# FrancisTheCat/raytracing_c

Measured on AMD Instinct MI355X. Metric: Mray/s, higher is better.
Workload: dtype f32; 1 GPU; helmet.glb 1920x1080, 256 spp, 8 bounces (BASELINE.json configs[2]); partition=single GPU

## Files before the change

### include/rt_hip.h

```cpp
#ifndef RT_HIP_H
#define RT_HIP_H

#include "rt_raytracer.h"
#include "rt_materials.h"

#ifdef __cplusplus
extern "C" {
#endif

extern char const *rt_last_error(void);
extern void        rt_clear_error(void);

extern int rt_init(int device);

extern int rt_set_devices(i32 n_devices, i32 rehearse);
extern i32 rt_device_count(void);


extern void rt_set_seed(u32 seed);
extern u32  rt_get_seed(void);


typedef struct RT_Device_Scene RT_Device_Scene;

// ... 88 lines not shown
#define RT_QUERY_MAX_RAYS ((i64)1 << 30)
extern int rt_query_closest(RT_Device_Scene *dscene, i64 n, void const *d_rays, void const *d_t_max, void *d_hits, void *d_full,
                            void *stream);
extern int rt_query_occluded(RT_Device_Scene *dscene, i64 n, void const *d_rays, void const *d_t_max, void *d_flags, void *stream);

#define RT_QUERY_SLICE ((i64)1 << 20)
extern int rt_scene_hits(Scene const *scene, i64 n, Ray const *rays, Hit *hits, i32 *triangles);
extern int rt_scene_closest(Scene const *scene, i64 n, Ray const *rays, f32 const *t_max, RT_Ray_Hit *hits);
extern int rt_scene_occluded(Scene const *scene, i64 n, Ray const *rays, f32 const *t_max, u8 *flags);

extern int rt_get_query_counters(RT_Query_Counters *out);


#define RT_FEATURE_CHANNELS 10
typedef struct { f32 *coverage, *albedo, *normal, *position; } RT_Features;

extern int rt_render_accumulate_features(RT_Device_Scene *dscene, RT_Render_Params const *params, void *d_sums, void *stream);
extern int rt_resolve_features(RT_Render_Params const *params, void const *d_sums,
                               void *d_coverage, void *d_albedo, void *d_normal, void *d_position, void *stream);
extern int rt_render_features(Scene const *scene, i32 width, i32 height, isize samples, isize max_bounces,
                              RT_Features const *out, u64 *sums);

#define RT_MOTION_CHANNELS 3
extern int rt_render_accumulate_features_motion(RT_Device_Scene *dscene, RT_Render_Params const *params, void *d_sums,
                                                void *d_motion_sums, void *stream);
extern int rt_resolve_motion(RT_Render_Params const *params, void const *d_motion_sums, void *d_motion, void *stream);
extern int rt_render_features_motion(Scene const *scene, i32 width, i32 height, isize samples, isize max_bounces,
                                     RT_Features const *out, u64 *sums, f32 *motion, u64 *motion_sums);


typedef struct {
  i32 iterations;
  f32 sigma_color, sigma_normal, sigma_position;
  i32 demodulate;
} RT_Guided_Params;

extern i64 rt_guided_work_bytes(i32 width, i32 height);
extern int rt_guided_denoise(i32 width, i32 height, RT_Guided_Params const *params, void const *d_color, void const *d_coverage,
                             void const *d_albedo, void const *d_normal, void const *d_position, void *d_out, void *d_image,
                             void *d_work, void *stream);
extern int rt_guided_denoise_host(i32 width, i32 height, RT_Guided_Params const *params, f32 const *color,
                                  RT_Features const *planes, f32 *out, u8 *image);
extern int rt_render_denoised(Scene const *scene, Image const *image, isize samples, isize max_bounces,
                              RT_Guided_Params const *params, f32 *linear_noisy, f32 *linear_denoised);


typedef struct {
  f32 alpha;
  i32 max_history;
  f32 normal_tolerance, plane_tolerance;
  i32 demodulate;
} RT_Temporal_Params;

typedef struct { f32 *color, *length, *coverage, *normal, *position; } RT_History_Planes;

extern i64 rt_temporal_history_bytes(i32 width, i32 height);
extern int rt_temporal_accumulate(i32 width, i32 height, RT_Temporal_Params const *params, Camera const *camera,
                                  Camera const *previous_camera, void const *d_color, void const *d_coverage, void const *d_albedo,
                                  void const *d_normal, void const *d_position, void const *d_history_in, void *d_history_out,
                                  void *d_out, void *d_length, void *d_image, void *stream);
extern int rt_temporal_accumulate_host(i32 width, i32 height, RT_Temporal_Params const *params, Camera const *camera,
                                       Camera const *previous_camera, f32 const *color, RT_Features const *planes,
                                       RT_History_Planes const *history_in, RT_History_Planes const *history_out, f32 *out,
                                       f32 *length, u8 *image);

typedef struct RT_History RT_History;
extern RT_History *rt_history_create(i32 width, i32 height);
extern int         rt_history_reset(RT_History *history);
extern void        rt_history_destroy(RT_History *history);
extern int         rt_history_set_motion(RT_History *history, int on);

extern int rt_render_temporal(Scene const *scene, Image const *image, isize samples, isize max_bounces, RT_History *history,
                              RT_Temporal_Params const *temporal_params, RT_Guided_Params const *guided_params, f32 *linear_noisy,
                              f32 *linear_out, f32 *length);


typedef struct { f32 sigma_normal, sigma_position; } RT_Variance_Params;

extern i64 rt_temporal_moments_bytes(i32 width, i32 height);
extern int rt_temporal_accumulate_moments(i32 width, i32 height, RT_Temporal_Params const *params, Camera const *camera,
                                          Camera const *previous_camera, void const *d_color, void const *d_coverage,
                                          void const *d_albedo, void const *d_normal, void const *d_position, void const *d_history_in,
                                          void *d_history_out, void *d_out, void *d_length, void *d_image, RT_Variance_Params const *vp,
                                          void const *d_moments_in, void *d_moments_out, void *d_variance, void *stream);
extern int rt_temporal_accumulate_moments_host(i32 width, i32 height, RT_Temporal_Params const *params, Camera const *camera,
                                               Camera const *previous_camera, f32 const *color, RT_Features const *planes,
                                               RT_History_Planes const *history_in, RT_History_Planes const *history_out, f32 *out,
                                               f32 *length, u8 *image, RT_Variance_Params const *vp, f32 const *moments_in,
                                               f32 *moments_out, f32 *variance);

extern int rt_temporal_accumulate_motion(i32 width, i32 height, RT_Temporal_Params const *params, Camera const *camera,
                                         Camera const *previous_camera, void const *d_color, void const *d_coverage,
                                         void const *d_albedo, void const *d_normal, void const *d_position, void const *d_history_in,
                                         void *d_history_out, void *d_out, void *d_length, void *d_image, RT_Variance_Params const *vp,
                                         void const *d_moments_in, void *d_moments_out, void *d_variance, void *stream,
                                         void const *d_motion);
extern int rt_temporal_accumulate_motion_host(i32 width, i32 height, RT_Temporal_Params const *params, Camera const *camera,
                                              Camera const *previous_camera, f32 const *color, RT_Features const *planes,
                                              RT_History_Planes const *history_in, RT_History_Planes const *history_out, f32 *out,
                                              f32 *length, u8 *image, RT_Variance_Params const *vp, f32 const *moments_in,
                                              f32 *moments_out, f32 *variance, f32 const *motion);

extern i64 rt_guided_variance_work_bytes(i32 width, i32 height);
extern int rt_guided_denoise_variance(i32 width, i32 height, RT_Guided_Params const *params, void const *d_color, void const *d_coverage,
                                      void const *d_albedo, void const *d_normal, void const *d_position, void *d_out, void *d_image,
                                      void *d_work, void *stream, void const *d_variance, void *d_variance_out);
extern int rt_guided_denoise_variance_host(i32 width, i32 height, RT_Guided_Params const *params, f32 const *color,
                                           RT_Features const *planes, f32 *out, u8 *image, f32 const *variance, f32 *variance_out);

extern int rt_render_svgf(Scene const *scene, Image const *image, isize samples, isize max_bounces, RT_History *history,
                          RT_Temporal_Params const *temporal_params, RT_Variance_Params const *variance_params,
                          RT_Guided_Params const *guided_params, f32 *linear_noisy, f32 *linear_out, f32 *length, f32 *variance);


typedef struct {
  f32 sigma_normal, sigma_position;
  i32 demodulate;
  i32 guide_samples;
} RT_Upsample_Params;

extern i64 rt_guided_upsample_work_bytes(i32 width, i32 height);
extern int rt_guided_upsample(i32 width, i32 height, RT_Upsample_Params const *params, void const *d_color_low,
                              void const *d_coverage_low, void const *d_albedo_low, void const *d_normal_low,
                              void const *d_position_low, void const *d_coverage, void const *d_albedo, void const *d_normal,
                              void const *d_position, void *d_out, void *d_image, void *d_work, void *stream);
extern int rt_guided_upsample_host(i32 width, i32 height, RT_Upsample_Params const *params, f32 const *color_low,
                                   RT_Features const *low, RT_Features const *full, f32 *out, u8 *image);
extern int rt_render_upsampled(Scene const *scene, Image const *image, isize samples, isize max_bounces,
                               RT_Upsample_Params const *upsample_params, RT_Guided_Params const *guided_params, f32 *linear_low,
                               f32 *linear_upsampled, f32 *linear_out);


extern int rt_render_accumulate_chunks(RT_Device_Scene *dscene, RT_Render_Params const *params, i32 n_list, i32 const *chunks,
                                       void *d_accum, void *stream);
extern int rt_adaptive_merge(i32 width, i32 height, i32 n, i32 n_list, i32 const *chunks, void *d_accum, void *d_fresh, void *d_err,
                             void *stream);
extern int rt_resolve_adaptive(i32 width, i32 height, void const *d_chunk_samples, void const *d_accum, void *d_image, void *d_linear,
                               void *d_sample_map, void *stream);

typedef struct {
  i32 min_samples;
  i32 max_samples;
  f32 threshold;
  i32 reserved;
} RT_Adaptive_Params;

extern int rt_render_adaptive(Scene const *scene, Image const *image, RT_Adaptive_Params const *ap, isize max_bounces, f32 *linear,
                              u64 *accum, i32 *chunk_samples);

extern int rt_get_counters(RT_Counters *out);
extern int rt_get_skipped_root_visits(u64 *out);
extern int rt_get_leafless_paths(u64 *out);
extern int rt_get_triangleless_paths(u64 *out);
extern int rt_get_fused_root_visits(u64 *out);
extern int rt_get_shade_taps_form(void);
extern int rt_materials_share_taps(f32 const *mats, i32 n_materials);

typedef struct {
  f32 stamp_ms, upload_ms, enqueue_ms, gpu_prep_ms, gpu_path_ms, gpu_resolve_ms, gpu_copy_ms, total_ms;
  f32 verify_ms;
  f32 gather_ms;
  i32 n_devices;
  i32 slowest_device;
} RT_Frame_Timing;
extern int rt_get_frame_timing(RT_Frame_Timing *out);

extern f32 rt_last_kernel_ms(void);

extern void rt_kernel_timing_reset(void);
extern f32  rt_kernel_timing_mean_ms(i32 *n_launches);

extern int rt_math_contract(void);


#ifdef __cplusplus
}
#endif

#endif
```

### raytracing_c_amd/csrc/rt_dev.hip.h

```cpp
#ifndef RT_DEV_HIP_H
#define RT_DEV_HIP_H

#include <hip/hip_runtime.h>
#include <stdint.h>

#include "rt_device.h"
#include "../../include/rt_math.h"

#define RT_BLOCK_WAVES 4
#define RT_BLOCK_THREADS (RT_BLOCK_WAVES * 64)

struct Ray3 {
  rt_v3 o, d;
  float inv_x, inv_y, inv_z;
  bool  fast;
};

__device__ __forceinline__ rt_v3 slab_bias3(const Ray3 &r) {
#ifdef RT_MATH_NO_FMA
  return rt_v3_make(0.0f, 0.0f, 0.0f);
#else
  float px, py, pz;
  asm volatile("v_mul_f32 %0, %1, %2" : "=v"(px) : "v"(r.o.x), "v"(r.inv_x));
  asm volatile("v_mul_f32 %0, %1, %2" : "=v"(py) : "v"(r.o.y), "v"(r.inv_y));
// ... 983 lines not shown
    emis = rt_v3_mul_add(s_emis, tint, emis);
    if (terminate) {
      done = true;
      radiance = emis;
    } else {
      dir = out_dir;
      tint = rt_v3_mul(tint, s_tint);
      float below = (rt_v3_dot(n_geo, out_dir) < 0.0f) ? 1.0f : 0.0f;
      float bias = (0.5f - below) * 2.0f * RT_EPS;
      org = rt_v3_madd(n_geo, bias, point);
    }
  }
  if (!done) {
    bounce += 1;
    if (bounce >= P.max_bounces) {
      done = true;
      radiance = emis;
    }
  }
  return done;
}

#define PH_NEED 0
#define PH_POP  1
#define PH_NODE 2
#define PH_LEAF 3
#define PH_HIT  4
#define PH_MISS 5

#define RT_PARK_FIELDS 18
#define RT_PARK_CAP 128
static_assert(RT_PARK_FIELDS * RT_PARK_CAP == RT_PARK_RECORD_DWORDS, "park slice size (rt_device.h) out of step");
#define RT_PARK_DENSE 48
#define RT_JOIN_CHOICES 4
#define RT_PYR_NUM 3
#define RT_PYR_DEN 4
#define RT_PYR_MIN 8
#define RT_STEAL_TRIES  16
#define RT_LEAF_CULL_MAX 4

__device__ __forceinline__ float *lds_at(float4 *smem, int byte_off) {
  asm volatile("" : "+s"(byte_off));
  return reinterpret_cast<float *>(reinterpret_cast<char *>(smem) + byte_off);
}
__device__ __forceinline__ int lane_now() {
  unsigned ones = ~0u;
  asm volatile("" : "+s"(ones));
  return (int)__builtin_amdgcn_mbcnt_hi(ones, __builtin_amdgcn_mbcnt_lo(ones, 0u));
}
__device__ __forceinline__ int lane_rank(unsigned long long mask) {
  return (int)__builtin_amdgcn_mbcnt_hi((uint32_t)(mask >> 32), __builtin_amdgcn_mbcnt_lo((uint32_t)mask, 0u));
}

template <int THREADS>
__device__ __forceinline__ void lds_load_nodes(float4 *smem, const float *nodes, int n_lds) {
  const float4 *g = reinterpret_cast<const float4 *>(nodes);
  for (int i = threadIdx.x; i < n_lds * RT_NODE_F4; i += THREADS) {
    int nd = i / RT_NODE_F4, q = i - nd * RT_NODE_F4;
    smem[nd * RT_LDS_NODE_F4 + q] = g[i];
  }
}

#define RT_LDS_PERM_LEVEL_F4 (RT_LDS_PERM_LEVEL_BYTES / 16)
#define RT_LDS_ACC_TILE_F4   (RT_LDS_ACC_TILE_BYTES / 16)
struct WaveLds {
  uint32_t *perm;
  unsigned long long *acc;
  int acc_off, pyr_off;
};
__device__ __forceinline__ int perm_stack_f4(int depth) { return (depth > 0 ? depth : 1) * RT_LDS_PERM_LEVEL_F4; }
__device__ __forceinline__ uint32_t *wave_perm(float4 *smem, int n_lds, int slice_f4, int wave) {
  return reinterpret_cast<uint32_t *>(smem + n_lds * RT_LDS_NODE_F4 + wave * slice_f4);
}
__device__ __forceinline__ WaveLds wave_lds(float4 *smem, int n_lds, int depth, int wave) {
  const int perm_f4 = perm_stack_f4(depth), slice_f4 = perm_f4 + RT_LDS_ACC_TILE_F4;
  const int base_f4 = n_lds * RT_LDS_NODE_F4 + __builtin_amdgcn_readfirstlane(wave) * slice_f4;
  WaveLds L;
  L.perm = wave_perm(smem, n_lds, slice_f4, wave);
  L.acc = reinterpret_cast<unsigned long long *>(reinterpret_cast<float4 *>(L.perm) + perm_f4);
  L.acc_off = (base_f4 + perm_f4) * 16;
  L.pyr_off = (base_f4 + perm_f4 - RT_LDS_PERM_LEVEL_F4) * 16;
  return L;
}
__device__ __forceinline__ void acc_tile_clear(unsigned long long *acc, const int lane) {
  acc[lane] = 0ull;
  acc[lane + 64] = 0ull;
  acc[lane + 128] = 0ull;
}
__device__ __forceinline__ void tile_add_sample(float4 *smem, const int acc_off, const int pixel, const rt_v3 radiance) {
  unsigned long long *ap = reinterpret_cast<unsigned long long *>(lds_at(smem, acc_off) + pixel * 6);
  atomicAdd(ap + 0, accum_quantize_dev(radiance.x));
  atomicAdd(ap + 1, accum_quantize_dev(radiance.y));
  atomicAdd(ap + 2, accum_quantize_dev(radiance.z));
}
#ifndef RT_SKY_ADD_GROUP
#define RT_SKY_ADD_GROUP 4
#endif
static_assert(RT_SKY_ADD_GROUP == 4 || RT_SKY_ADD_GROUP == 16 || RT_SKY_ADD_GROUP == 64, "RT_SKY_ADD_GROUP: 4, 16 or 64");
template <int CTRL>
__device__ __forceinline__ unsigned long long dpp_u64(const unsigned long long v) {
  typedef uint32_t u32x2 __attribute__((ext_vector_type(2)));
  u32x2 p = __builtin_bit_cast(u32x2, v);
  p.x = (uint32_t)__builtin_amdgcn_mov_dpp((int)p.x, CTRL, 0xF, 0xF, true);
  p.y = (uint32_t)__builtin_amdgcn_mov_dpp((int)p.y, CTRL, 0xF, 0xF, true);
  return __builtin_bit_cast(unsigned long long, p);
}
template <int CTRL>
__device__ __forceinline__ void dpp_add3_u64(unsigned long long &r, unsigned long long &g, unsigned long long &b) {
  const unsigned long long pr = dpp_u64<CTRL>(r), pg = dpp_u64<CTRL>(g), pb = dpp_u64<CTRL>(b);
  r += pr; g += pg; b += pb;
}
__device__ __forceinline__ unsigned long long rows_sum_u64(unsigned long long v) {
  typedef uint32_t u32x2 __attribute__((ext_vector_type(2)));
  u32x2 p = __builtin_bit_cast(u32x2, v);
  const auto l16 = __builtin_amdgcn_permlane16_swap(p.x, p.x, false, false), h16 = __builtin_amdgcn_permlane16_swap(p.y, p.y, false, false);
  u32x2 a = {l16[0], h16[0]}, b = {l16[1], h16[1]};
  v = __builtin_bit_cast(unsigned long long, a) + __builtin_bit_cast(unsigned long long, b);
  p = __builtin_bit_cast(u32x2, v);
  const auto l32 = __builtin_amdgcn_permlane32_swap(p.x, p.x, false, false), h32 = __builtin_amdgcn_permlane32_swap(p.y, p.y, false, false);
  a = u32x2{l32[0], h32[0]}; b = u32x2{l32[1], h32[1]};
  return __builtin_bit_cast(unsigned long long, a) + __builtin_bit_cast(unsigned long long, b);
}
template <int G>
__device__ __forceinline__ void group_sum3_u64(unsigned long long &r, unsigned long long &g, unsigned long long &b) {
  static_assert(G == 4 || G == 16 || G == 64, "group_sum3_u64: groups of 4, 16 or 64 lanes");
  dpp_add3_u64<0xB1>(r, g, b);
  dpp_add3_u64<0x4E>(r, g, b);
  if (G >= 16) {
    dpp_add3_u64<0x141>(r, g, b);
    dpp_add3_u64<0x140>(r, g, b);
  }
  if (G >= 64) { r = rows_sum_u64(r); g = rows_sum_u64(g); b = rows_sum_u64(b); }
}
__device__ __forceinline__ void lds_add_u64_noret(const uint32_t at, const unsigned long long r, const unsigned long long g,
                                                  const unsigned long long b) {
  asm volatile("ds_add_u64 %0, %1\n\tds_add_u64 %0, %2 offset:8\n\tds_add_u64 %0, %3 offset:16" : : "v"(at), "v"(r), "v"(g), "v"(b) : "memory");
}
__device__ __forceinline__ void tile_add_samples_grouped(float4 *smem, const int acc_off, const int pixel, const bool grouped, const bool has,
                                                         unsigned long long r, unsigned long long g, unsigned long long b) {
  bool adds = true;
  if (grouped) {
    group_sum3_u64<RT_SKY_ADD_GROUP>(r, g, b);
    adds = (lane_now() & (RT_SKY_ADD_GROUP - 1)) == 0;
  }
  if (adds && has) {
    const uint32_t at = (uint32_t)(uintptr_t)(__attribute__((address_space(3))) float *)lds_at(smem, acc_off) + (uint32_t)pixel * 24u;
    lds_add_u64_noret(at, r, g, b);
  }
}
#define RT_PYR_PLANE      0
#define RT_PYR_ORIGIN     16
#define RT_PYR_ROOT_POP   19
#define RT_PYR_ROOT_FUSED 20
#define RT_PYR_LEAF_CACHE 24
#define RT_PYR_NODE_CACHE 32
#define RT_PYR_CACHE_WORDS 40

__device__ __forceinline__ bool child_box_empty(float mnx, float mny, float mnz, float mxx, float mxy, float mxz) {
  return mnx == 0.0f && mny == 0.0f && mnz == 0.0f && mxx == 0.0f && mxy == 0.0f && mxz == 0.0f;
}
__device__ __forceinline__ bool child_box_empty(const float *nb) { return child_box_empty(nb[0], nb[8], nb[16], nb[24], nb[32], nb[40]); }

__device__ __forceinline__ uint32_t pyramid_cull_mask(const float4 *lds_nodes, const float *pyr, int node) {
  const int lane = lane_now();
  const float *nb = reinterpret_cast<const float *>(lds_nodes + lds_node_f4(node)) + (lane & 7);
  const float *pl = pyr + RT_PYR_PLANE + ((lane >> 3) & 3) * 4;
  const float ox = pyr[RT_PYR_ORIGIN], oy = pyr[RT_PYR_ORIGIN + 1], oz = pyr[RT_PYR_ORIGIN + 2];
  const float mnx = nb[0], mny = nb[8], mnz = nb[16], mxx = nb[24], mxy = nb[32], mxz = nb[40];
  const float nx = pl[0], ny = pl[1], nz = pl[2];
  const bool empty = child_box_empty(mnx, mny, mnz, mxx, mxy, mxz);
  const float lox = nx * (mnx - ox), hix = nx * (mxx - ox), loy = ny * (mny - oy), hiy = ny * (mxy - oy);
  const float loz = nz * (mnz - oz), hiz = nz * (mxz - oz);
  const float nearest = fminf(lox, hix) + fminf(loy, hiy) + fminf(loz, hiz);
  const float extent = fmaxf(fabsf(lox), fabsf(hix)) + fmaxf(fabsf(loy), fabsf(hiy)) + fmaxf(fabsf(loz), fabsf(hiz));
  const float coarse = fabsf(nx) * (fabsf(ox) + fmaxf(fabsf(mnx), fabsf(mxx))) + fabsf(ny) * (fabsf(oy) + fmaxf(fabsf(mny), fabsf(mxy))) +
                       fabsf(nz) * (fabsf(oz) + fmaxf(fabsf(mnz), fabsf(mxz)));
  const bool outside = empty || nearest > 1e-3f * extent + 1e-6f * coarse;
  const uint32_t m = (uint32_t)__ballot(outside);
  return (m | (m >> 8) | (m >> 16) | (m >> 24)) & 0xFFu;
}

__device__ __forceinline__ float slab_entry_ordered(const Ray3 &r, const rt_v3 &bs, const char *nbase, int k, int nx, int ny, int nz, float t_max) {
  const char *b = nbase + k * 4;
  const float sx = rt_slab_t_fast(*reinterpret_cast<const float *>(b + nx), r.o.x, r.inv_x, bs.x);
  const float bx = rt_slab_t_fast(*reinterpret_cast<const float *>(b + (96 - nx)), r.o.x, r.inv_x, bs.x);
  const float sy = rt_slab_t_fast(*reinterpret_cast<const float *>(b + 32 + ny), r.o.y, r.inv_y, bs.y);
  const float by = rt_slab_t_fast(*reinterpret_cast<const float *>(b + 32 + (96 - ny)), r.o.y, r.inv_y, bs.y);
  const float sz = rt_slab_t_fast(*reinterpret_cast<const float *>(b + 64 + nz), r.o.z, r.inv_z, bs.z);
  const float bz = rt_slab_t_fast(*reinterpret_cast<const float *>(b + 64 + (96 - nz)), r.o.z, r.inv_z, bs.z);
  const float t_minv = fmax_hw(RT_EPS, fmax_hw(sx, fmax_hw(sy, sz)));
  const float t_maxv = fmin_hw(t_max, fmin_hw(bx, fmin_hw(by, bz)));
  return (t_minv < t_maxv) ? t_minv : RT_INF;
}

#define LGM_FEW(name) do { if (AT_ROOT) LGM("rfew_" name); else LGM("nfew_" name); } while (0)
template <bool AT_ROOT = false>
__device__ __forceinline__ uint32_t node_enter_few(const Ray3 &r, const float4 *lds_nodes, int node, uint32_t surv,
                                                   float hit_t) {
  const char *nbase = reinterpret_cast<const char *>(lds_nodes + lds_node_f4(node));
  const int nx = (as_i(r.inv_x) >> 31) & 96, ny = (as_i(r.inv_y) >> 31) & 96, nz = (as_i(r.inv_z) >> 31) & 96;
  const rt_v3 bs = slab_bias3(r);
  const int n = (int)__popc(surv);
  const int k0 = (int)__builtin_ctz(surv);
  const int e0 = as_i(slab_entry_ordered(r, bs, nbase, k0, nx, ny, nz, hit_t));
  const uint32_t f0 = 1u - (((uint32_t)e0 + 0x00800000u) >> 31);
  LGM_FEW("ret1");
  if (n == 1) return (uint32_t)k0 | (f0 << 24);
  surv &= surv - 1u;
  const int k1 = (int)__builtin_ctz(surv);
  const int e1 = as_i(slab_entry_ordered(r, bs, nbase, k1, nx, ny, nz, hit_t));
  const uint32_t f1 = 1u - (((uint32_t)e1 + 0x00800000u) >> 31);
  LGM_FEW("two");
  if (n == 2) {
    const bool swap = e1 < e0;
    const uint32_t first = swap ? (uint32_t)k1 : (uint32_t)k0, second = swap ? (uint32_t)k0 : (uint32_t)k1;
    return first | (second << 3) | ((f0 + f1) << 24);
  }
  LGM_FEW("ret2");
  surv &= surv - 1u;
  const int k2 = (int)__builtin_ctz(surv);
  const int e2 = as_i(slab_entry_ordered(r, bs, nbase, k2, nx, ny, nz, hit_t));
  const uint32_t f2 = 1u - (((uint32_t)e2 + 0x00800000u) >> 31);
  int e3 = 0x7F800000, k3 = 0;
  uint32_t f3 = 0;
  LGM_FEW("four_begin");
  if (n == 4) {
    surv &= surv - 1u;
    k3 = (int)__builtin_ctz(surv);
      e3 = as_i(slab_entry_ordered(r, bs, nbase, k3, nx, ny, nz, hit_t));
    f3 = 1u - (((uint32_t)e3 + 0x00800000u) >> 31);
  }
  LGM_FEW("four_end");
  const int e[4] = {e0, e1, e2, e3};
  const int kk[4] = {k0, k1, k2, k3};
  int rank[4] = {0, 1, 2, 3};
#pragma unroll
  for (int j = 0; j < 4; j++) {
#pragma unroll
    for (int k = j + 1; k < 4; k++) {
      int kb = (int)((uint32_t)(e[k] - e[j]) >> 31);
      rank[j] += kb;
      rank[k] -= kb;
    }
  }
  uint32_t w = 0;
#pragma unroll
  for (int j = 0; j < 4; j++) w |= (uint32_t)kk[j] << (3 * rank[j]);
  return w | ((f0 + f1 + f2 + f3) << 24);
}
#undef LGM_FEW

template <bool PADDING = false>
__device__ __forceinline__ uint32_t pyramid_cull_tris(const float *leaves, const float *pyr, int g, uint32_t *padding = nullptr) {
  const int lane = lane_now();
  const float *tb = leaves + (size_t)g * 72 + (lane & 7);
  const float *pl = pyr + RT_PYR_PLANE + ((lane >> 3) & 3) * 4;
  const float ox = pyr[RT_PYR_ORIGIN], oy = pyr[RT_PYR_ORIGIN + 1], oz = pyr[RT_PYR_ORIGIN + 2];
  const float nx = pl[0], ny = pl[1], nz = pl[2];
  const float ax = tb[0], e1x = tb[8], e2x = tb[16], ay = tb[24], e1y = tb[32], e2y = tb[40], az = tb[48], e1z = tb[56], e2z = tb[64];
  const float band = 2.5f * RT_EPS * (fabsf(nx * e1x + ny * e1y + nz * e1z) + fabsf(nx * e2x + ny * e2y + nz * e2z));
  bool outside = true;
#pragma unroll
  for (int v = 0; v < 3; v++) {
    const float vx = v == 0 ? ax : (v == 1 ? ax + e1x : ax + e2x);
    const float vy = v == 0 ? ay : (v == 1 ? ay + e1y : ay + e2y);
    const float vz = v == 0 ? az : (v == 1 ? az + e1z : az + e2z);
    const float px = nx * (vx - ox), py = ny * (vy - oy), pz = nz * (vz - oz);
    const float val = px + py + pz;
    const float extent = fabsf(px) + fabsf(py) + fabsf(pz);
    const float coarse = fabsf(nx) * (fabsf(ox) + fabsf(vx)) + fabsf(ny) * (fabsf(oy) + fabsf(vy)) + fabsf(nz) * (fabsf(oz) + fabsf(vz));
    outside = outside && (val - band > 1e-3f * extent + 1e-6f * coarse);
  }
  const uint32_t m = (uint32_t)__ballot(outside);
  if (PADDING) {
    const bool zero = ax == 0.0f && e1x == 0.0f && e2x == 0.0f && ay == 0.0f && e1y == 0.0f && e2y == 0.0f && az == 0.0f && e1z == 0.0f && e2z == 0.0f;
    *padding = (uint32_t)__ballot(zero) & 0xFFu;
  }
  return (m | (m >> 8) | (m >> 16) | (m >> 24)) & 0xFFu;
}

template <bool SHORT_DIV>
__device__ __forceinline__ void tri_test_uniform(const Ray3 &r, rt_v3 a, rt_v3 edge1, rt_v3 edge2, int k, float &best, float &bu, float &bv, int &bi) {
  rt_v3 rxe2 = rt_v3_cross(r.d, edge2);
  float det = rt_v3_dot(edge1, rxe2);
  float inv_det = SHORT_DIV ? rcp_leaf(det) : 1.0f / det;
  rt_v3 s = rt_v3_sub(r.o, a);
  rt_v3 sxe1 = rt_v3_cross(s, edge1);
  float u = inv_det * rt_v3_dot(s, rxe2);
  float v = inv_det * rt_v3_dot(r.d, sxe1);
  float t = inv_det * rt_v3_dot(edge2, sxe1);
  bool miss = (u < -RT_EPS) || (u > 1.0f + RT_EPS) || (v < -RT_EPS) || (u + v > 1.0f + RT_EPS) || (t < RT_EPS);
  if (SHORT_DIV) {
    if (!miss && t < best) { best = t; bi = k; bu = u; bv = v; }
  } else {
    float dist = miss ? RT_INF : t;
    dist = (dist > 0.0f) ? dist : RT_INF;
    if (dist < best) { best = dist; bi = k; bu = u; bv = v; }
  }
}
template <bool SHORT_DIV>
__device__ __forceinline__ bool leaf_test_uniform(const RT_KParams &P, const Ray3 &r, int g, uint32_t surv, HitRec &hit) {
  float best = RT_INF, bu = 0.0f, bv = 0.0f;
  int   bi = 0;
  cfloat *lb = as_scalar_ptr(P.leaves) + (size_t)g * 72;
  while (surv) {
    const int k0 = (int)__builtin_ctz(surv);
// ... 340 lines not shown
```

### raytracing_c_amd/csrc/rt_device.h

```cpp
#ifndef RT_DEVICE_H
#define RT_DEVICE_H

#include <stdint.h>

#define RT_NODE_F4   12
#define RT_LEAF_F4   18
#define RT_TRI_F4     7
#define RT_MAT_F4     9
#define RT_MAT_FLOATS 36
#define RT_MAX_DEPTH  8

#define RT_LDS_BYTES            (160 * 1024)
#define RT_LDS_NODE_BYTES       208
#define RT_LDS_TABLE_BYTES      64
#define RT_LDS_PERM_LEVEL_BYTES 256
#define RT_LDS_ACC_TILE_BYTES   1536

#define RT_MAT_DISNEY 0
#define RT_MAT_DEBUG  1

#define RT_TILE      8
#define RT_TILE_PIX  64

#define RT_PARK_RECORD_DWORDS (18 * 128)
enum {
  RT_CNT_PATHS = 0, RT_CNT_RAYS, RT_CNT_NODES, RT_CNT_LEAVES, RT_CNT_SHADES, RT_CNT_BG, RT_CNT_TEXTURED,
  RT_CNT_SKIPPED_ROOT,
  RT_CNT_LEDGER,
  RT_CNT_LEAFLESS = 136,
  RT_CNT_FUSED_ROOT,
  RT_CNT_TRIANGLELESS,
  RT_N_COUNTERS
};
#define RT_CNT_LEDGER_SLOTS (RT_CNT_LEAFLESS - RT_CNT_LEDGER)



typedef struct {
  uint32_t offset;
  int32_t  width, height, stride;
} RT_DTexture;
#define RT_TEX_TILE_INDEX(x, y, tpr) ((((y) >> 2) * (tpr) + ((x) >> 2)) * 16 + (((y) & 3) << 2) + ((x) & 3))

typedef struct RT_KView {
  float    cam[3][4];
  float    focal_length;
  uint32_t seed;
  uint32_t pad[2];
} RT_KView;

typedef struct {
  const float    *nodes;
  const float    *leaves;
  const float    *tris;
  const float    *mats;
  const RT_DTexture *textures;
  const uint32_t *texels;
  int32_t depth;
  int32_t last_row_offset;
  int32_t bg_texture;
  int32_t n_nodes;
  float cam[3][4];
  float focal_length;
  float inv_width, inv_height, aspect;
  int32_t width, height, samples, max_bounces;
  int32_t sample_first, sample_end;
  uint32_t seed;
  int32_t chunks_x, n_chunks;
  int32_t rank, world, n_local_chunks;
  int32_t shared_taps;
  int32_t unused_pad[2];
  int32_t sched_thresh;
  int32_t n_lds_nodes;
  unsigned long long *accum;
  unsigned long long *counters;
  uint32_t *work_head;
  const int32_t *local_chunks;
  const uint32_t *order;
  uint32_t *tile_cost;
  unsigned long long *wave_times;
  uint32_t *tile_next;
  uint32_t *open_groups;
  int32_t n_tiles;
  int32_t chunk_shift;
  int32_t n_chunks_tile;
  int32_t n_sample_blocks;
  int32_t drain_thresh;
  int32_t grab_max;
  uint32_t *park;
  int32_t short_div;
  int32_t pyr_nodes;
  uint32_t *wf_hit0;
  uint32_t *wf_hit;
  uint32_t *wf_ray[2];
  uint32_t *wf_cnt_hit0, *wf_cnt_hit, *wf_cnt_ray[2];
  uint32_t *wf_ctl;
  int32_t wf_soft_chunks;
  int32_t wf_bounce;
  int32_t wf_n_waves;
  const RT_KView *views;
  int32_t n_views;
  int32_t tiles_per_view;
  int32_t pixels_per_view;
} RT_KParams;

typedef struct {
  const float *rays;
  const float *t_max;
  float       *hits;
  uint8_t     *flags;
  uint32_t    *head;
  unsigned long long *counters;
  int32_t      n;
  int32_t      grab;
  int32_t      exit_lanes;
} RT_QParams;
enum { RT_QCNT_RAYS = 0, RT_QCNT_HITS, RT_QCNT_NODES, RT_QCNT_LEAVES, RT_QUERY_COUNTERS };
#define RT_HIT_DWORDS     22

typedef struct {
  unsigned long long *sums;
  uint32_t    *head;
  int32_t      n_units;
  int32_t      grab;
  int32_t      tiles_x;
  int32_t      shift;
  int32_t      n_sample_blocks;
  int32_t      units_per_tile;
} RT_FParams;

typedef struct {
  float r[3][3];
  float t[3];
  float focal_length;
} RT_TCamera;
typedef struct {
  RT_TCamera cur, prev;
  int32_t width, height;
  float   half_w, half_h;
  float   aspect;
  float   tn2, tp2;
  float   alpha;
  float   max_history;
  int32_t demodulate;
  int32_t tiles_x;
} RT_TParams;

typedef struct {
  const float *color, *coverage, *albedo, *normal, *position;
} RT_Frame;

#define WF_CHUNK        256
#define WF_HIT0_FIELDS  9
#define WF_HIT_FIELDS   5
#define WF_RAY_FIELDS   15
#define WF_CTL_STRIDE   16
enum {
  WF_HIT0_ALLOC = 0, WF_HIT0_HEAD, WF_HIT_ALLOC, WF_HIT_HEAD, WF_RAY0_ALLOC, WF_RAY0_HEAD, WF_RAY1_ALLOC, WF_RAY1_HEAD,
  WF_STOPPED,
  WF_DONE_WAVES,
  WF_N_CTL
};

#endif
```

### raytracing_c_amd/csrc/rt_kernels.hip

```cpp

#include "rt_dev.hip.h"


#ifdef RT_LEDGER
#define RT_LEDGER_WAVES 8192
__device__ uint32_t g_ledger[RT_LEDGER_WAVES * RT_LEDGER_ROW];
__global__ void rt_ledger_reduce_kernel(unsigned long long *counters) {
  const int slot = threadIdx.x;
  if (slot >= LG_N || slot >= RT_LEDGER_ROW) return;
  unsigned long long sum = 0ull;
  for (int w = 0; w < RT_LEDGER_WAVES; w++) sum += g_ledger[w * RT_LEDGER_ROW + slot];
  counters[RT_CNT_LEDGER + slot] = sum;
}
#endif

template <int WAVES, bool LDSN, int MIN_WAVES_PER_SIMD, bool SHORT_DIV, bool VIEWS, bool SHARED_TAPS>
__global__ __launch_bounds__(WAVES * 64, MIN_WAVES_PER_SIMD) void rt_path_kernel_stream(RT_KParams P) {
  extern __shared__ float4 smem[];
  const int lane = threadIdx.x & 63;
  const int wave = threadIdx.x >> 6;
  const int n_lds = LDSN ? P.n_lds_nodes : 0;
  const float4 *lds_nodes = smem;
  const WaveLds L = wave_lds(smem, n_lds, P.depth, wave);
  unsigned long long *acc = L.acc;
  const int acc_off = L.acc_off, pyr_off = L.pyr_off;

#ifdef RT_LEDGER
  uint32_t *lg = g_ledger + (size_t)__builtin_amdgcn_readfirstlane((int)blockIdx.x * WAVES + wave) * RT_LEDGER_ROW;
  const unsigned long long lg_wave_t0 = __builtin_amdgcn_s_memtime();
#if RT_LEDGER >= 2
  unsigned long long lg_drain_t0 = 0ull;
#endif
#endif
  pow24_lds_init((int)threadIdx.x);
  if (LDSN) {
    LGT0();
    lds_load_nodes<WAVES * 64>(smem, P.nodes, n_lds);
    __syncthreads();
    LGT1(LG_CYC_COPY);
  } else {
    __syncthreads();
  }

  acc_tile_clear(acc, lane);

  if (LDSN) {
    uint32_t *pw = reinterpret_cast<uint32_t *>(lds_at(smem, pyr_off));
    bool populated = false;
    if (lane_now() < 8 && cold_args()->n_lds_nodes > 0 && cold_args()->depth > 0) {
      populated = !child_box_empty(lds_at(smem, 0) + lane_now());
    }
    const uint32_t pm = (uint32_t)__ballot(populated) & 0xFFu;
#ifdef RT_ROOT_AT_NODE_BLOCKS
    if (lane_now() == 0) { pw[RT_PYR_ROOT_POP] = 0u; pw[RT_PYR_ROOT_FUSED] = 0u; }
#else
    if (lane_now() == 0) { pw[RT_PYR_ROOT_POP] = __popc(pm) <= 4 ? pm : 0u; pw[RT_PYR_ROOT_FUSED] = 0u; }
#endif
  }

  uint32_t w_paths = 0, w_rays = 0, w_nodes = 0, w_leaves = 0, w_shades = 0, w_bgs = 0, w_tex = 0;
  const unsigned long long t_wave_start = cold_args()->wave_times ? __builtin_amdgcn_s_memrealtime() : 0ull;
  uint32_t n_tiles_done = 0;
  unsigned long long t_last_grab = 0ull;

  const int shift = P.chunk_shift;
  const int unit_paths = 2 << shift;
  const uint32_t n_chunks_tile = (uint32_t)P.n_chunks_tile;
  const int leaf_level = P.depth - 1;
  const int thresh = P.sched_thresh;
  const int drain_thresh = P.drain_thresh;
  const int pyr_nodes = LDSN ? P.pyr_nodes : 0;
  const int wave_id = (int)blockIdx.x * WAVES + wave;

  bool queue_open = true;
  int  steal_tries = 0;

  for (;;) {
    LGT0();
    LGM("tile_begin");
    int tile_idx = queue_open ? take_queue_tile(lane, queue_open) : -1;
    if (tile_idx < 0) {
      if (steal_tries >= RT_STEAL_TRIES) break;
      steal_tries += 1;
      LG(LG_JOIN_X, 1);
      tile_idx = join_open_tile(lane, wave_id, steal_tries, n_chunks_tile LG_ARG);
      if (tile_idx < 0) break;
    }

    int tile_x0, tile_y0;
    RT_KViewP vrec = nullptr;
    if (!tile_origin<VIEWS>(lane, tile_idx, n_chunks_tile, tile_x0, tile_y0, vrec)) continue;
    bool tile_root_miss = false;
    if (leaf_level >= 0) {
      typename CamSrc<VIEWS>::type S;
      if constexpr (VIEWS) S = vrec; else S = cold_args();
      tile_root_miss = tile_pyramid(S, P.nodes, smem, pyr_off, lane, tile_x0, tile_y0);
    }
    int n_list = 0;
    int ll_levels = leaf_level, ll_nodes = pyr_nodes, ll_leaf0 = P.last_row_offset;
    asm volatile("" : "+s"(ll_levels), "+s"(ll_nodes), "+s"(ll_leaf0));
    if (ll_levels >= 1 && ll_nodes > 0 && !tile_root_miss) n_list = leafless_walk(smem, lds_nodes, pyr_off, ll_levels, ll_nodes, ll_leaf0, cold_args()->leaves);
    const uint32_t rays_before = w_rays;
    LG(LG_TILE_X, 1);
    LGM("tile_end");
    LGT1(LG_CYC_TILE);

    int   pix = 0, bounce = 0;
    uint32_t rng = 0;
    Ray3  ray;
    ray_setup(ray, rt_v3_make(0, 0, 0), rt_v3_make(0, 0, 1));
    rt_v3 tint = rt_v3_make(1, 1, 1), emis = rt_v3_make(0, 0, 0);
    TravState T = RT_TRAV_IDLE;

    bool tile_open = true;
    TileUnits U;
    tile_units_init(U, queue_open);
    int  n_parked = 0;
    uint32_t *park = cold_args()->park;

    if ((tile_root_miss || n_list > 0) && cold_args()->max_bounces > 0) {
      RT_KArgs A = cold_args();
      typename CamSrc<VIEWS>::type S;
      if constexpr (VIEWS) S = vrec; else S = A;
      const int width = A->width, height = A->height, sample_first = A->sample_first, sample_end = A->sample_end;
      const uint32_t n_sb = (uint32_t)A->n_sample_blocks, gmax = (uint32_t)A->grab_max;
      PrimaryParams PP;
      primary_params(PP, S, A);
      ShadeParamsLds SP;
      shade_params(SP, A, false);
      uint32_t *tile_next = A->tile_next, *open_groups = A->open_groups;
      uint32_t n_sky = 0;
      const uint32_t *list = leafless_list(smem, pyr_off, ll_levels);
      const uint32_t list_entry = (n_list > 1 && lane_now() < n_list) ? list[RT_LL_ENTRY + (lane_now() & 31)] : 0u;
      for (;;) {
        if (U.c_next >= U.c_end) {
          if (U.u_cur + 1u < U.u_end) {
            U.u_cur += 1u;
          } else {
            uint32_t u0 = 0;
            if (lane == 0) u0 = atomicAdd(&tile_next[tile_idx], U.grab);
            u0 = (uint32_t)__builtin_amdgcn_readfirstlane((int)u0);
            if (u0 >= n_chunks_tile) { tile_open = false; break; }
            U.u_cur = u0;
            U.u_end = u0 + U.grab < n_chunks_tile ? u0 + U.grab : n_chunks_tile;
            if (U.u_end == n_chunks_tile && lane == 0) atomicSub(&open_groups[tile_idx >> 6], 1u);
            if (t_wave_start) t_last_grab = __builtin_amdgcn_s_memrealtime();
            LG(LG_GRAB_X, 1);
            const uint32_t left = n_chunks_tile - U.u_end;
            U.grab = left >= 8u * gmax ? gmax : (left >= 8u && gmax >= 2u ? 2u : 1u);
            U.took_any = true;
          }
          unit_decode(U, tile_x0, tile_y0, shift, unit_paths, n_sb, sample_first, width, height);
          continue;
        }
#ifndef RT_SKY_PATHS
#define RT_SKY_PATHS 1
#endif
        LGM("sky_begin");
        LGT0();
        const int avail = U.c_end - U.c_next;
        const int take = avail < 64 * RT_SKY_PATHS ? avail : 64 * RT_SKY_PATHS;
        const int l = lane_now();
        bool valid[RT_SKY_PATHS];
        int  pxs[RT_SKY_PATHS];
        rt_v3 dirs[RT_SKY_PATHS];
        Ray3 rs[RT_SKY_PATHS];
        bool slow = false;
#pragma unroll
        for (int q = 0; q < RT_SKY_PATHS; q++) {
          const int kq = l + 64 * q;
          const int k = U.c_next + kq;
          pxs[q] = k >> shift;
          const int sm = U.c_s0 + (k & ((1 << shift) - 1));
          const int x = U.c_x0 + pxs[q];
          valid[q] = kq < take && x < width && sm < sample_end;
          rt_v3 o = rt_v3_make(0, 0, 0);
          dirs[q] = rt_v3_make(0, 0, 1);
          if (valid[q]) primary_ray(PP, x, U.c_y, sm, o, dirs[q]);
          ray_setup<SHORT_DIV>(rs[q], o, dirs[q]);
          slow = slow || (valid[q] && !rs[q].fast);
        }
        if (__ballot(slow) != 0ull) break;
        uint32_t nv = 0;
        uint32_t e = (uint32_t)__builtin_amdgcn_readlane((int)list_entry, 1);
        if ((int)e < 0) {
#pragma unroll
          for (int q = 0; q < RT_SKY_PATHS; q++) {
            const Ray3 &r = rs[q];
            const int nx = (as_i(r.inv_x) >> 31) & 96, ny = (as_i(r.inv_y) >> 31) & 96, nz = (as_i(r.inv_z) >> 31) & 96;
            const rt_v3 bs = slab_bias3(r);
            uint32_t entered = valid[q] ? 1u : 0u;
            int i = 1;
            if (q > 0) e = (uint32_t)__builtin_amdgcn_readlane((int)list_entry, 1);
            do {
              const char *cb = reinterpret_cast<const char *>(lds_nodes) + (e & 0xFFFFFu);
              const float t = slab_entry_ordered(r, bs, cb, 0, nx, ny, nz, RT_INF);
              const uint32_t in = ((entered >> ((e >> 20) & 31u)) & 1u) & (t < RT_INF ? 1u : 0u);
              entered |= in << i;
              const uint32_t n_in = (uint32_t)__popcll(__ballot(in != 0u));
              if (e & RT_LL_GROUP) w_leaves += n_in;
              else w_nodes += n_in;
              i += 1;
              e = (uint32_t)__builtin_amdgcn_readlane((int)list_entry, i);
            } while ((int)e < 0);
          }
        }
#pragma unroll
        for (int q = 0; q < RT_SKY_PATHS; q++) {
          unsigned long long qr = 0ull, qg = 0ull, qb = 0ull;
          if (valid[q]) {
            const rt_v3 bg = background_lookup(SP, dirs[q]);
            const rt_v3 radiance = rt_v3_mul_add(bg, rt_v3_make(1, 1, 1), rt_v3_make(0, 0, 0));
            qr = accum_quantize_dev(radiance.x); qg = accum_quantize_dev(radiance.y); qb = accum_quantize_dev(radiance.z);
          }
          tile_add_samples_grouped(smem, acc_off, U.c_pix0 + pxs[q], U.c_end >= 2 * RT_SKY_ADD_GROUP, valid[q], qr, qg, qb);
          nv += (uint32_t)__popcll(__ballot(valid[q]));
        }
        w_paths += nv; w_rays += nv; w_nodes += nv; w_bgs += nv;
        n_sky += nv;
        LG(LG_SKY_X, 1); LG(LG_SKY_L, nv);
        U.c_next += take;
        LGT1(LG_CYC_SKY);
        LGM("sky_end");
      }
      if (n_sky != 0u && lane == 0) atomicAdd(cold_args()->counters + (tile_root_miss ? RT_CNT_SKIPPED_ROOT : RT_CNT_LEAFLESS), (unsigned long long)n_sky);
      if (n_sky != 0u && (__ballot((list_entry & RT_LL_GROUP) != 0u) & ~1ull) != 0ull && lane == 0)
        atomicAdd(cold_args()->counters + RT_CNT_TRIANGLELESS, (unsigned long long)n_sky);
    }

    for (;;) {
      {
        LGT0();
        LGM("s_begin");
        LG(LG_S_ITER, 1);
        LaneCounters cn;
        cn.rays = cn.nodes = cn.leaves = cn.shades = cn.bgs = cn.textured = cn.paths = 0;
        bool  done = false, start = false, fresh = false;
        rt_v3 radiance = rt_v3_make(0, 0, 0);
        rt_v3 org = ray.o, dir = ray.d;
        RT_KArgs A = cold_args();
        typename PathShadeParams<SHARED_TAPS>::type SP;
        shade_params(SP, A, true);
#ifdef RT_LEDGER
        { const int n_env = (int)__popcll(__ballot(T.phase == PH_MISS)); LG(LG_ENV_X, n_env != 0); LG(LG_ENV_L, n_env); }
#endif
        LGM("env_begin");
        if (T.phase == PH_MISS) {
          cn.bgs = 1;
          rt_v3 bg = background_lookup(SP, dir);
          radiance = rt_v3_mul_add(bg, tint, emis);
          done = true;
        }
        LGM("env_end");
        bool shade_now = true;
        if (park) {
          const unsigned long long mHit = __ballot(T.phase == PH_HIT);
          const unsigned long long mIdle = __ballot(T.phase == PH_NEED) | __ballot(T.phase == PH_MISS);
          const int h = (int)__popcll(mHit), f = (int)__popcll(mIdle);
          const int back = n_parked < f ? n_parked : f;
          uint32_t *pk = park + (size_t)__builtin_amdgcn_readfirstlane(wave_id) * (RT_PARK_FIELDS * RT_PARK_CAP);
          if (!tile_open || h + back >= RT_PARK_DENSE || n_parked + h > RT_PARK_CAP) {
            if (back > 0) {
              LG(LG_PLOAD_X, 1); LG(LG_PLOAD_L, back);
              LGM("pload_begin");
              if (done) {
                tile_add_sample(smem, acc_off, pix, radiance);
                T.phase = PH_NEED;
                done = false;
              }
              const int rank = lane_rank(mIdle);
              if (T.phase == PH_NEED && rank < back) {
                const uint32_t *q = pk + (n_parked - 1 - rank);
                uint32_t v[RT_PARK_FIELDS];
                __builtin_amdgcn_fence(__ATOMIC_ACQUIRE, "wavefront");
#pragma unroll
                for (int i = 0; i < RT_PARK_FIELDS; i++)
                  v[i] = __hip_atomic_load(q + i * RT_PARK_CAP, __ATOMIC_RELAXED, __HIP_MEMORY_SCOPE_AGENT);
                T.hit.t = as_f((int)v[0]); T.hit.tri = (int)v[1]; T.hit.u = as_f((int)v[2]); T.hit.v = as_f((int)v[3]);
                org = rt_v3_make(as_f((int)v[4]), as_f((int)v[5]), as_f((int)v[6]));
                dir = rt_v3_make(as_f((int)v[7]), as_f((int)v[8]), as_f((int)v[9]));
                tint = rt_v3_make(as_f((int)v[10]), as_f((int)v[11]), as_f((int)v[12]));
                emis = rt_v3_make(as_f((int)v[13]), as_f((int)v[14]), as_f((int)v[15]));
                rng = v[16]; pix = (int)(v[17] & 63u); bounce = (int)(v[17] >> 6);
                T.phase = PH_HIT;
              }
              n_parked -= back;
              LGM("pload_end");
            }
          } else if (h > 0) {
            LG(LG_PSTORE_X, 1); LG(LG_PSTORE_L, h);
            LGM("pstore_begin");
            shade_now = false;
            const int rank = lane_rank(mHit);
            if (T.phase == PH_HIT) {
              uint32_t *q = pk + (n_parked + rank);
              const uint32_t v[RT_PARK_FIELDS] = {(uint32_t)as_i(T.hit.t), (uint32_t)T.hit.tri, (uint32_t)as_i(T.hit.u), (uint32_t)as_i(T.hit.v),
                                                  (uint32_t)as_i(org.x), (uint32_t)as_i(org.y), (uint32_t)as_i(org.z),
                                                  (uint32_t)as_i(dir.x), (uint32_t)as_i(dir.y), (uint32_t)as_i(dir.z),
                                                  (uint32_t)as_i(tint.x), (uint32_t)as_i(tint.y), (uint32_t)as_i(tint.z),
                                                  (uint32_t)as_i(emis.x), (uint32_t)as_i(emis.y), (uint32_t)as_i(emis.z),
                                                  rng, (uint32_t)pix | ((uint32_t)bounce << 6)};
#pragma unroll
              for (int i = 0; i < RT_PARK_FIELDS; i++) q[i * RT_PARK_CAP] = v[i];
              __builtin_amdgcn_fence(__ATOMIC_RELEASE, "wavefront");
              T.phase = PH_NEED;
            }
            n_parked += h;
            LGM("pstore_end");
          }
        }
#ifdef RT_LEDGER
        { const int n_sh = (int)__popcll(__ballot(T.phase == PH_HIT && shade_now)); LG(LG_SHADE_X, n_sh != 0); LG(LG_SHADE_L, n_sh); }
#endif
        LGM("shade_begin");
        if (T.phase == PH_HIT && shade_now) {
          done = shade_hit(SP, T.hit, org, dir, tint, emis, rng, bounce, cn, radiance);
          start = !done;
        }
        LGM("shade_end");
#ifdef RT_LEDGER
        { const int n_acc = (int)__popcll(__ballot(done)); LG(LG_ACCUM_X, n_acc != 0); LG(LG_ACCUM_L, n_acc); }
#endif
        LGM("accum_begin");
        if (done) {
          tile_add_sample(smem, acc_off, pix, radiance);
          T.phase = PH_NEED;
        }
        LGM("accum_end");
        w_shades += (uint32_t)__popcll(__ballot(cn.shades != 0));
        w_tex += (uint32_t)__popcll(__ballot(cn.textured != 0));
        w_bgs += (uint32_t)__popcll(__ballot(cn.bgs != 0));

        if (tile_open) {
          NewPath np = {0, 0, 0, 0};
          const bool got = regen_paths(T.phase, np, SP.max_bounces > 0, U, tile_open, false, lane, tile_idx, n_chunks_tile, tile_x0, tile_y0,
                                       shift, unit_paths, t_wave_start, t_last_grab, w_paths LG_ARG);
          if (!tile_open) LGD0((int)__popcll(__ballot(T.phase != PH_NEED || got)) + n_parked);
          const int gx = np.x, gy = np.y, gs = np.sample, width = A->width;
#ifdef RT_LEDGER
          { const int n_pr = (int)__popcll(__ballot(got)); LG(LG_PRIM_X, n_pr != 0); LG(LG_PRIM_L, n_pr); LG(LG_REGEN_L, n_pr); }
#endif
          LGM("prim_begin");
          if (got) {
            typename CamSrc<VIEWS>::type S;
            if constexpr (VIEWS) S = vrec; else S = A;
            pix = np.pix;
            bounce = 0;
            rng = rt_path_seed(S->seed, (uint32_t)(gx + gy * width), (uint32_t)gs);
            PrimaryParams PP;
            primary_params(PP, S, A);
            primary_ray(PP, gx, gy, gs, org, dir);
            tint = rt_v3_make(1, 1, 1);
            emis = rt_v3_make(0, 0, 0);
            start = true;
            fresh = true;
          }
          LGM("prim_end");
        }
        bool skip_root = false;
#ifdef RT_LEDGER
        { const int n_st = (int)__popcll(__ballot(start)); LG(LG_START_X, n_st != 0); LG(LG_START_L, n_st); }
#endif
        LGM("start_begin");
        if (start) {
          ray_setup<SHORT_DIV>(ray, org, dir);
          trav_start(T, leaf_level, P.last_row_offset);
          T.cur = (LDSN && ray.fast && reinterpret_cast<const uint32_t *>(lds_at(smem, pyr_off))[RT_PYR_ROOT_POP] != 0u) ? 1u : 0u;
          skip_root = fresh && tile_root_miss && ray.fast;
          if (skip_root) T.phase = PH_MISS;
        }
        LGM("start_end");
        w_rays += (uint32_t)__popcll(__ballot(start));
        {
          const uint32_t n_skip = (uint32_t)__popcll(__ballot(skip_root));
          w_nodes += n_skip;
          if (n_skip != 0u && lane == 0) atomicAdd(cold_args()->counters + RT_CNT_SKIPPED_ROOT, (unsigned long long)n_skip);
        }
        LGM("s_end");
        LGT1(LG_CYC_S);
      }

      const int n_trav0 = (int)__popcll(__ballot(T.phase == PH_NODE || T.phase == PH_LEAF));
      if (n_trav0 == 0) {
        if (__any(T.phase == PH_MISS)) continue;
        if (n_parked > 0 || __any(T.phase == PH_HIT)) continue;
        if (!tile_open) break;
        continue;
      }

      if (LDSN) {
        const bool at_root = T.phase == PH_NODE && T.level < 0 && T.cur != 0u;
        const int n_root = (int)__popcll(__ballot(at_root));
        if (n_root != 0) {
          LGM("root_begin");
          LG(LG_ROOTF_X, 1); LG(LG_ROOTF_L, n_root);
          uint32_t *pw = reinterpret_cast<uint32_t *>(lds_at(smem, pyr_off));
          const uint32_t w_pop = pw[RT_PYR_ROOT_POP], w_cull = pw[RT_PYR_NODE_CACHE];
          uint32_t rsurv = (uint32_t)__builtin_amdgcn_readfirstlane((int)w_pop);
          w_nodes += (uint32_t)n_root;
          if (lane_now() == 0) {
            const uint32_t at = (uint32_t)(uintptr_t)(__attribute__((address_space(3))) uint32_t *)(pw + RT_PYR_ROOT_FUSED);
            asm volatile("ds_add_u32 %0, %1" : : "v"(at), "v"((uint32_t)n_root) : "memory");
          }
          if (__ballot(at_root && bounce != 0) == 0ull) {
            const uint32_t ce = (uint32_t)__builtin_amdgcn_readfirstlane((int)w_cull);
            if ((ce >> 8) == 1u) rsurv &= ~ce;
          }
          if (at_root) {
            T.level = 0;
            T.cur = rsurv ? node_enter_few<true>(ray, lds_nodes, 0, rsurv, RT_INF) : 0u;
            if (T.cur >> 24) {
              T.child = 1 + (int)(T.cur & 7u);
              T.cur = ((T.cur >> 3) & 0x1FFFFFu) | (((T.cur >> 24) - 1u) << 24);
              T.phase = (leaf_level == 0) ? PH_LEAF : PH_NODE;
            } else {
              T.level = -1;
              T.phase = PH_MISS;
            }
          }
          LGM("root_end");
        }
      }

      const TravWave W = {smem, lds_nodes, L.perm, n_lds, pyr_nodes, pyr_off, leaf_level, lane};
      traversal_blocks<LDSN, SHORT_DIV, true>(P, W, ray, bounce == 0, T, tile_open ? thresh : drain_thresh, n_trav0, w_nodes, w_leaves LG_ARG);
    }

    LGD1();
    LGM("flush_begin");
    if (U.took_any) {
      LGT0();
      LG(LG_FLUSH_X, 1);
      RT_KArgs A = cold_args();
      unsigned long long *frame = A->accum;
      if constexpr (VIEWS) frame += (size_t)(vrec - (RT_KViewP)A->views) * (size_t)A->pixels_per_view * 3;
      flush_tile(acc, lane, tile_x0, tile_y0, frame, tile_idx, w_rays - rays_before);
      if (LDSN && lane == 0) {
        uint32_t *pw = reinterpret_cast<uint32_t *>(lds_at(smem, pyr_off));
        const uint32_t n_fused = pw[RT_PYR_ROOT_FUSED];
        pw[RT_PYR_ROOT_FUSED] = 0u;
        if (n_fused != 0u) atomicAdd(A->counters + RT_CNT_FUSED_ROOT, (unsigned long long)n_fused);
      }
      steal_tries = 0;
      n_tiles_done += 1;
      LGT1(LG_CYC_FLUSH);
    }
  }
  RT_KArgs A = cold_args();
  unsigned long long *wave_times = A->wave_times, *counters = A->counters;
  if (wave_times && lane == 0 && wave_id < 65536) {
    wave_times[wave_id * 3 + 0] = t_wave_start;
    wave_times[wave_id * 3 + 1] = __builtin_amdgcn_s_memrealtime();
    wave_times[wave_id * 3 + 2] = ((t_last_grab - t_wave_start) << 16) | (n_tiles_done & 0xFFFFu);
  }

  if (lane == 0) {
    atomicAdd(counters + RT_CNT_PATHS, (unsigned long long)w_paths);
    atomicAdd(counters + RT_CNT_RAYS, (unsigned long long)w_rays);
    atomicAdd(counters + RT_CNT_NODES, (unsigned long long)w_nodes);
    atomicAdd(counters + RT_CNT_LEAVES, (unsigned long long)w_leaves);
    atomicAdd(counters + RT_CNT_SHADES, (unsigned long long)w_shades);
    atomicAdd(counters + RT_CNT_BG, (unsigned long long)w_bgs);
    atomicAdd(counters + RT_CNT_TEXTURED, (unsigned long long)w_tex);
#ifdef RT_LEDGER
    LG(LG_CYC_WAVE, (uint32_t)((__builtin_amdgcn_s_memtime() - lg_wave_t0) >> 4));
#endif
  }
}

__global__ void rt_resolve_kernel(int width, int height, int samples, int chunks_x, const int32_t *local_chunks,
                                  int n_local_chunks, const unsigned long long *accum,
                                  uint8_t *tiles, uint8_t *image, float *linear) {
  int idx = blockIdx.x * blockDim.x + threadIdx.x;
  if (idx >= n_local_chunks * 1024) return;
  int lchunk = idx >> 10, p = idx & 1023;
  int chunk = local_chunks[lchunk];
  int x = (chunk % chunks_x) * 32 + (p & 31);
  int y = (chunk / chunks_x) * 32 + (p >> 5);
  uint8_t rgb[3] = {0, 0, 0};
  if (x < width && y < height) {
    size_t pix = (size_t)y * width + x;
#pragma unroll
    for (int c = 0; c < 3; c++) {
      float lin = rt_accum_resolve(accum[pix * 3 + c], (uint32_t)samples);
      if (linear) linear[pix * 3 + c] = lin;
      rgb[c] = rt_encode_u8(lin);
      if (image) image[pix * 3 + c] = rgb[c];
    }
  }
// ... 440 lines not shown
```

### raytracing_c_amd/csrc/rt_launch.cpp

```cpp

#include "rt_host.h"

static std::atomic<int> g_taps_form{-1};

int check_params(RT_Render_Params const *p) {
  if (!p) return rt_fail("render params are NULL");
  if (p->width <= 0 || p->height <= 0) return rt_fail("image size %dx%d is invalid", p->width, p->height);
  if ((int64_t)p->width * p->height > (int64_t)1 << 28) return rt_fail("image %dx%d is too large", p->width, p->height);
  if (p->samples <= 0) return rt_fail("samples must be positive (got %d)", p->samples);
  if (p->max_bounces < 0) return rt_fail("max_bounces must be >= 0 (got %d)", p->max_bounces);
  if (p->world <= 0 || p->rank < 0 || p->rank >= p->world) return rt_fail("rank %d / world %d is invalid", p->rank, p->world);
  if (p->sample_first < 0 || p->sample_count < 0 || p->sample_first + p->sample_count > p->samples)
    return rt_fail("sample range [%d, +%d) outside [0, %d)", p->sample_first, p->sample_count, p->samples);
  return 0;
}

int check_image_size(const char *who, i32 width, i32 height) {
  if (width <= 0 || height <= 0) return rt_fail("%s: image size %dx%d is invalid", who, width, height);
  if ((int64_t)width * height > RT_MAX_PIXELS) return rt_fail("%s: image %dx%d is too large (more than 2^28 pixels)", who, width, height);
  return 0;
}

int check_views(i32 n_views, RT_View const *views, i32 width, i32 height, const char *who) {
  if (n_views <= 0) return rt_fail("%s: n_views must be positive (got %d)", who, n_views);
// ... 91 lines not shown
  if (batch) {
    K->n_views = nv;
    K->tiles_per_view = K->n_local_chunks * 16;
    K->pixels_per_view = p->width * p->height;
  }
  return 0;
}

static void launch_geometry(const Device &D, const RT_Device_Scene *d, RT_KParams &K, int *wg_waves, int *smem) {
  const int64_t paths = (int64_t)K.n_tiles * 64 * (int64_t)(K.sample_end - K.sample_first);
  int64_t per_slot = paths / ((int64_t)D.num_cus * 16 * 64);
  if (K.depth == 0) per_slot /= 4;
  *wg_waves = per_slot < 12 ? 8 : (per_slot < 40 ? 12 : 16);
  int v = knob_int("RT_WG_WAVES", 0);
  if (v == 8 || v == 12 || v == 16) *wg_waves = v;
  LdsSplit S = lds_split(d, K.depth, *wg_waves, RT_LDS_ACC_TILE_BYTES, 1, true);
  S.cap(knob_int("RT_LDS_NODES", -1));
  K.n_lds_nodes = S.n_lds_nodes;
  *smem = S.smem;
}

static int schedule_feedback(LaunchState &L, RT_KParams &K, const uint32_t **cost_prev) {
  K.order = nullptr;
  K.tile_cost = nullptr;
  *cost_prev = nullptr;
  if (knob_is("RT_ORDER", "identity") || K.n_tiles <= 0) return 0;
  const int n_tiles = K.n_tiles;
  uint64_t key = 1469598103934665603ull;
  auto mix = [&key](const void *ptr, size_t n) {
    const unsigned char *b = (const unsigned char *)ptr;
    for (size_t i = 0; i < n; i++) { key ^= b[i]; key *= 1099511628211ull; }
  };
  int32_t ids[6] = {K.width, K.height, K.rank, K.world, K.max_bounces, n_tiles};
  mix(ids, sizeof ids);
  if (L.sched_tiles != n_tiles) {
    L.cost[0].reset(); L.cost[1].reset(); L.order.reset();
    L.sched_tiles = 0;
    L.sched_valid = false;
    HIP_TRY(L.cost[0].grow((size_t)n_tiles));
    HIP_TRY(L.cost[1].grow((size_t)n_tiles));
    HIP_TRY(L.order.grow((size_t)n_tiles));
    L.sched_tiles = n_tiles;
  }
  if (L.sched_valid && L.sched_key == key) {
    *cost_prev = L.cost[L.sched_cur ^ 1];
    K.order = L.order;
  }
  K.tile_cost = L.cost[L.sched_cur];
  L.sched_cur ^= 1;
  L.sched_key = key;
  L.sched_valid = true;
  return 0;
}

static int upload_view_table(LaunchState &L, RT_KParams &K, ViewBatch const *batch, hipStream_t stream) {
  const int nv = batch->n;
  HIP_TRY(L.views.grow((size_t)nv));
  HIP_TRY(L.views_host.grow((size_t)nv));
  if (!L.views_copied) HIP_TRY(L.views_copied.ensure(hipEventDisableTiming));
  else HIP_TRY(hipEventSynchronize(L.views_copied));
  for (int v = 0; v < nv; v++) {
    RT_KView &r = L.views_host[v];
    memset(&r, 0, sizeof r);
    camera_rows(r.cam, &batch->views[v].camera);
    r.focal_length = batch->views[v].camera.focal_length;
    r.seed = batch->views[v].seed;
  }
  HIP_TRY(hipMemcpyAsync(L.views, L.views_host, (size_t)nv * sizeof(RT_KView), hipMemcpyHostToDevice, stream));
  HIP_TRY(hipEventRecord(L.views_copied, stream));
  K.views = L.views;
  return 0;
}

int stage_chunk_list(ChunkListStage &S, ChunkList const &list, hipStream_t stream, const int32_t **d_list) {
  if (!S.copied) HIP_TRY(S.copied.ensure(hipEventDisableTiming));
  else HIP_TRY(hipEventSynchronize(S.copied));
  if (S.dev && S.dev.cap < (size_t)list.n) HIP_TRY(hipStreamSynchronize(stream));
  HIP_TRY(S.dev.grow((size_t)list.n));
  HIP_TRY(S.host.grow((size_t)list.n));
  if (list.n > 0) {
    memcpy(S.host.get(), list.chunks, (size_t)list.n * sizeof(int32_t));
    HIP_TRY(hipMemcpyAsync(S.dev, S.host, (size_t)list.n * sizeof(int32_t), hipMemcpyHostToDevice, stream));
    HIP_TRY(hipEventRecord(S.copied, stream));
  }
  *d_list = S.dev;
  return 0;
}

int render_accumulate_locked(Device &D, RT_Device_Scene *d, Camera const *cam, RT_Render_Params const *p, void *d_accum,
                             hipStream_t stream, hipEvent_t ev_prep, int launch_state, ViewBatch const *batch, ChunkList const *list) {
  if (ensure_device(D) != 0) return -1;
  if (check_params(p) != 0) return -1;
  if (!d || !d_accum) return rt_fail("rt_render_accumulate: NULL scene or accumulation buffer");
  if (d->dev != &D) return rt_fail("rt_render_accumulate: the scene was uploaded to another device");
  if (batch && check_views(batch->n, batch->views, p->width, p->height, "view batch") != 0) return -1;
  if (list && (batch || launch_state != RT_ADAPTIVE_STATE || p->rank != 0 || p->world != 1 ||
               check_chunk_list("chunk list", p->width, p->height, list->n, list->chunks) != 0))
    return rt_fail("rt_render_accumulate: a chunk list needs rank 0 of 1, no view batch, its own launch state and a valid list");
  const int nv = batch ? batch->n : 1;
  RT_KParams K;
  if (fill_kparams(D, &K, d, cam, p, d_accum, batch, list) != 0) return -1;
  if (launch_state < 0 || launch_state > RT_ADAPTIVE_STATE) return rt_fail("rt_render_accumulate: launch state %d out of range", launch_state);
  if (!list && launch_state == RT_ADAPTIVE_STATE) return rt_fail("rt_render_accumulate: launch state %d serves chunk lists only", launch_state);
  LaunchState &L = d->ls[launch_state];
  HIP_TRY(L.counters.grow(RT_N_COUNTERS));
  HIP_TRY(L.work_head.grow(16));
  K.counters = L.counters;
  K.work_head = L.work_head;
  D.last_counters = L.counters;
  bool wavefront = false;
#ifdef RT_DIAG_VARIANTS
  wavefront = g_pipeline.load() == 1 || knob_is("RT_PIPELINE", "wf");
#endif
  if (batch && wavefront) return rt_fail("view batch: a batch of views needs the tile-stream path kernel (the wavefront pipeline is set)");

  int wg_waves, smem;
  launch_geometry(D, d, K, &wg_waves, &smem);
  int waves_per_cu = knob_int("RT_WAVES_PER_CU", 0);
  if (waves_per_cu <= 0) waves_per_cu = wg_waves;
  K.sched_thresh = knob_int("RT_SCHED_THRESH", 48);
  if (K.sched_thresh < 1 || K.sched_thresh > 64) K.sched_thresh = 48;
  K.drain_thresh = knob_int("RT_DRAIN_THRESH", K.sched_thresh);
  if (K.drain_thresh < 1 || K.drain_thresh > 64) K.drain_thresh = K.sched_thresh;

  const uint32_t *cost_prev = nullptr;
  K.order = nullptr;
  K.tile_cost = nullptr;
  if (!list && schedule_feedback(L, K, &cost_prev) != 0) return -1;

  const int n_samples = K.sample_end - K.sample_first;
  const int cs = p->slab > 0 ? p->slab : 64;
  int cshift = 0;
  while ((1 << cshift) < cs && (1 << cshift) < n_samples) cshift++;
  K.chunk_shift = cshift;
  K.n_sample_blocks = (n_samples + (1 << cshift) - 1) >> cshift;
  K.n_chunks_tile = 32 * K.n_sample_blocks;
  const int tiles_room = list ? K.n_chunks * 16 : K.n_tiles;
  if (L.tile_next_n < tiles_room) {
    L.tile_next_n = 0;
    HIP_TRY(L.tile_next.grow((size_t)tiles_room + (size_t)((tiles_room + 63) / 64)));
    L.tile_next_n = tiles_room;
  }
  K.tile_next = L.tile_next;
  K.open_groups = L.tile_next + L.tile_next_n;
  const int64_t n_units = (int64_t)K.n_tiles * K.n_chunks_tile;
  int n_waves = D.num_cus * waves_per_cu;
  if ((int64_t)n_waves > n_units) n_waves = (int)n_units;
  K.grab_max = (cshift >= 6 || (int64_t)K.n_tiles < (int64_t)2 * n_waves) ? 1 : 2;
  {
    int v = knob_int("RT_GRAB", 0);
    if (v == 1 || v == 2 || v == 4) K.grab_max = v;
  }
  K.pyr_nodes = knob_int("RT_PYRAMID", 1) ? K.n_lds_nodes : 0;
  float cam_max = 0.0f;
  for (int v = 0; v < nv; v++)
    for (int i = 0; i < 3; i++)
      for (int j = 0; j < 3; j++) {
        float m = fabsf(batch ? batch->views[v].camera.view_matrix.rows[i][j] : K.cam[i][j]);
        if (!(m <= cam_max)) cam_max = m;
      }
  K.short_div = (d->max_edge <= 0x1p38f && cam_max <= 0x1p16f) ? 1 : 0;
  if (knob_int("RT_SHORT_DIV", 1) == 0) K.short_div = 0;
  K.shared_taps = (d->shared_taps && knob_int("RT_SHARED_TAPS", 1) != 0) ? 1 : 0;
  K.park = nullptr;
  if (!wavefront && knob_int("RT_PARK", 1) != 0 && K.max_bounces < (1 << 26)) {
    const int grid_waves = (n_waves + wg_waves - 1) / wg_waves * wg_waves;
    const size_t slice_dwords = RT_PARK_RECORD_DWORDS;
    HIP_TRY(L.park.grow((size_t)grid_waves * slice_dwords));
    K.park = L.park;
  }

  K.views = nullptr;
  if (batch && upload_view_table(L, K, batch, stream) != 0) return -1;
  if (list && stage_chunk_list(L.list, *list, stream, &K.local_chunks) != 0) return -1;

  {
    int rc2 = rt_launch_prepare(K.n_tiles, K.tile_next, K.open_groups, L.counters, L.work_head, K.tile_cost, cost_prev,
                                cost_prev ? L.order : nullptr, stream);
    if (rc2 != 0) return rt_fail("prepare kernel launch failed: %s", hipGetErrorString((hipError_t)rc2));
  }
  if (ev_prep) HIP_TRY(hipEventRecord(ev_prep, stream));
  if (n_units == 0) return 0;

  K.wave_times = nullptr;
  if (knob_set("RT_WAVE_TIMES")) {
    HIP_TRY(D.ws.wave_times.grow((size_t)65536 * 3));
    HIP_TRY(hipMemsetAsync(D.ws.wave_times, 0, (size_t)65536 * 3 * 8, stream));
    K.wave_times = D.ws.wave_times;
    if (n_waves > 65536) n_waves = 65536;
    D.ws.wave_times_n = n_waves;
  }

  size_t slot = D.ws.n_timed % RT_MAX_TIMED;
  if (slot >= D.ws.ev0.size()) {
    D.ws.ev0.emplace_back();
    D.ws.ev1.emplace_back();
  }
  HIP_TRY(D.ws.ev0[slot].ensure());
  HIP_TRY(D.ws.ev1[slot].ensure());
  HIP_TRY(hipEventRecord(D.ws.ev0[slot], stream));
#ifdef RT_DIAG_VARIANTS
  if (wavefront) {
    if (launch_wavefront(D, d, K, stream) != 0) return -1;
  } else
#endif
  {
    int rc = rt_launch_path_kernel(&K, n_waves, smem, wg_waves, stream);
    if (rc != 0) return rt_fail("path kernel launch failed: %s", hipGetErrorString((hipError_t)rc));
    g_taps_form.store(K.shared_taps);
  }
  HIP_TRY(hipEventRecord(D.ws.ev1[slot], stream));
  D.ws.n_timed += 1;
  return 0;
}

extern "C" int rt_set_camera(RT_Device_Scene *dscene, Camera const *camera) {
  if (!dscene || !camera) return rt_fail("rt_set_camera: NULL argument");
  Device &D = *dscene->dev;
  std::lock_guard<std::mutex> lock(D.mutex);
  D.cameras[dscene] = *camera;
  return 0;
}

extern "C" int rt_render_accumulate(RT_Device_Scene *dscene, RT_Render_Params const *params, void *d_accum,
                                    void *stream) {
  if (!dscene) return rt_fail("rt_render_accumulate: NULL scene or accumulation buffer");
  Device &D = *dscene->dev;
  std::lock_guard<std::mutex> lock(D.mutex);
  DeviceGuard guard(D);
  auto it = D.cameras.find(dscene);
  if (it == D.cameras.end()) return rt_fail("rt_render_accumulate: no camera set for this scene (rt_set_camera)");
  forget_multi_counters();
  return render_accumulate_locked(D, dscene, &it->second, params, d_accum, (hipStream_t)stream);
}

extern "C" int rt_render_accumulate_chunks(RT_Device_Scene *dscene, RT_Render_Params const *params, i32 n_list, i32 const *chunks,
                                           void *d_accum, void *stream) {
  const char *who = "rt_render_accumulate_chunks";
  if (!dscene || !d_accum) return rt_fail("%s: NULL scene or accumulation buffer", who);
  if (check_params(params) != 0) return -1;
  if (params->world != 1 || params->rank != 0)
    return rt_fail("%s: a chunk list replaces the partition: rank 0 of world 1 only (got %d of %d)", who, params->rank, params->world);
  if (check_chunk_list(who, params->width, params->height, n_list, chunks) != 0) return -1;
  Device &D = *dscene->dev;
  std::lock_guard<std::mutex> lock(D.mutex);
  DeviceGuard guard(D);
  auto it = D.cameras.find(dscene);
  if (it == D.cameras.end()) return rt_fail("%s: no camera set for this scene (rt_set_camera)", who);
  forget_multi_counters();
  ChunkList list;
  list.n = n_list;
  list.chunks = chunks;
  return render_accumulate_locked(D, dscene, &it->second, params, d_accum, (hipStream_t)stream, nullptr, RT_ADAPTIVE_STATE, nullptr, &list);
}

extern "C" int rt_render_accumulate_views(RT_Device_Scene *dscene, RT_Render_Params const *params, i32 n_views,
                                          RT_View const *views, void *d_accum, void *stream) {
  if (!dscene || !d_accum) return rt_fail("rt_render_accumulate_views: NULL scene or accumulation buffer");
  if (check_params(params) != 0) return -1;
  if (check_views(n_views, views, params->width, params->height, "rt_render_accumulate_views") != 0) return -1;
  Device &D = *dscene->dev;
  std::lock_guard<std::mutex> lock(D.mutex);
  DeviceGuard guard(D);
  forget_multi_counters();
  ViewBatch batch;
  batch.n = n_views;
  batch.views = views;
  return render_accumulate_locked(D, dscene, &views[0].camera, params, d_accum, (hipStream_t)stream, nullptr, RT_VIEWS_STATE, &batch);
}

int resolve_on(Device &D, RT_Render_Params const *p, void const *d_accum, void *d_tiles, void *d_image, void *d_linear,
               hipStream_t stream) {
  if (check_params(p) != 0) return -1;
  if (!d_accum) return rt_fail("rt_resolve: NULL accumulation buffer");
  int chunks_x = (p->width + RT_CHUNK_SIZE - 1) / RT_CHUNK_SIZE;
  const int32_t *d_list = nullptr;
  int n_local = 0;
  if (device_chunk_list(D, p->width, p->height, p->rank, p->world, &d_list, &n_local) != 0) return -1;
  int rc = rt_launch_resolve(p->width, p->height, p->samples, chunks_x, d_list, n_local,
                             (const unsigned long long *)d_accum, (uint8_t *)d_tiles, (uint8_t *)d_image,
                             (float *)d_linear, stream);
  if (rc != 0) return rt_fail("resolve kernel launch failed: %s", hipGetErrorString((hipError_t)rc));
  return 0;
}

extern "C" int rt_resolve(RT_Render_Params const *p, void const *d_accum, void *d_tiles, void *d_image,
                          void *d_linear, void *stream) {
  Device &D = dev0();
  {
    std::lock_guard<std::mutex> lock(D.mutex);
    if (ensure_device(D) != 0) return -1;
  }
  return resolve_on(D, p, d_accum, d_tiles, d_image, d_linear, (hipStream_t)stream);
}

int untile_on(Device &D, i32 width, i32 height, i32 world, void const *d_all_tiles, void *d_image, hipStream_t stream) {
  if (width <= 0 || height <= 0 || world <= 0 || !d_all_tiles || !d_image) return rt_fail("rt_untile: bad arguments");
  int chunks_x = (width + RT_CHUNK_SIZE - 1) / RT_CHUNK_SIZE;
  const int32_t *d_table = nullptr;
  int n_chunks = 0;
  if (!partition_args_ok(width, height, world)) return rt_fail("rt_untile: bad arguments");
  if (device_owner_table(D, width, height, world, &d_table, &n_chunks) != 0) return -1;
  int rc = rt_launch_untile(width, height, chunks_x, n_chunks, d_table, (const uint8_t *)d_all_tiles,
                            (uint8_t *)d_image, stream);
  if (rc != 0) return rt_fail("untile kernel launch failed: %s", hipGetErrorString((hipError_t)rc));
  return 0;
}

extern "C" int rt_untile(i32 width, i32 height, i32 world, void const *d_all_tiles, void *d_image, void *stream) {
  Device &D = dev0();
  {
    std::lock_guard<std::mutex> lock(D.mutex);
    if (ensure_device(D) != 0) return -1;
  }
  return untile_on(D, width, height, world, d_all_tiles, d_image, (hipStream_t)stream);
}

int ensure_ws_buffers(Workspace &W, int width, int height, size_t tiles_bytes, size_t all_tiles_bytes, bool want_linear) {
  const size_t pixels = (size_t)width * height;
  HIP_TRY(W.accum.grow(pixels * 3));
  HIP_TRY(W.image.grow(pixels * 3));
  if (want_linear) HIP_TRY(W.linear.grow(pixels * 3));
  if (tiles_bytes) HIP_TRY(W.tiles.grow(tiles_bytes));
  if (all_tiles_bytes) HIP_TRY(W.all_tiles.grow(all_tiles_bytes));
  for (DevEvent &e : W.ev_frame) HIP_TRY(e.ensure());
  return 0;
}

int copy_image_out(Image const *image, const uint8_t *d_image, int width, int height, hipStream_t stream) {
  size_t pixels = (size_t)width * height;
  if (!image->pixels.data) return 0;
  if (image->components == 3 && image->stride == image->width) {
    HIP_TRY(hipMemcpyAsync(image->pixels.data, d_image, pixels * 3, hipMemcpyDeviceToHost, stream));
    HIP_TRY(hipStreamSynchronize(stream));
  } else {
    std::vector<uint8_t> tmp(pixels * 3);
    HIP_TRY(hipMemcpy(tmp.data(), d_image, pixels * 3, hipMemcpyDeviceToHost));
    for (isize y = 0; y < image->height; y++)
      for (isize x = 0; x < image->width; x++)
        for (int c = 0; c < 3; c++)
          image->pixels.data[image->components * (x + y * image->stride) + c] = tmp[((size_t)y * width + x) * 3 + c];
  }
  return 0;
}

static int get_counter(const char *who, int index, u64 *out) {
  if (!out) return rt_fail("%s: NULL", who);
  Device &D = dev0();
  std::lock_guard<std::mutex> lock(D.mutex);
  if (ensure_device(D) != 0) return -1;
  unsigned long long c[RT_N_COUNTERS];
  if (read_counters(D, c) != 0) return -1;
  *out = c[index];
  return 0;
}

extern "C" int rt_get_skipped_root_visits(u64 *out) { return get_counter("rt_get_skipped_root_visits", RT_CNT_SKIPPED_ROOT, out); }

extern "C" int rt_get_leafless_paths(u64 *out) { return get_counter("rt_get_leafless_paths", RT_CNT_LEAFLESS, out); }

extern "C" int rt_get_triangleless_paths(u64 *out) { return get_counter("rt_get_triangleless_paths", RT_CNT_TRIANGLELESS, out); }

extern "C" int rt_get_fused_root_visits(u64 *out) { return get_counter("rt_get_fused_root_visits", RT_CNT_FUSED_ROOT, out); }

extern "C" int rt_get_shade_taps_form(void) { return g_taps_form.load(); }

int read_counters(Device &D, unsigned long long c[RT_N_COUNTERS]) {
  HIP_TRY(hipDeviceSynchronize());
  if (!D.last_counters) { memset(c, 0, RT_N_COUNTERS * sizeof(unsigned long long)); return 0; }
  HIP_TRY(hipMemcpy(c, D.last_counters, RT_N_COUNTERS * sizeof(unsigned long long), hipMemcpyDeviceToHost));
  return 0;
}

extern "C" int rt_get_counters(RT_Counters *out) {
  if (!out) return rt_fail("rt_get_counters: NULL");
  {
    std::lock_guard<std::mutex> lk(g_multi_mutex);
    if (g_multi_counters_valid) { *out = g_multi_counters; return 0; }
  }
  Device &D = dev0();
  std::lock_guard<std::mutex> lock(D.mutex);
  if (ensure_device(D) != 0) return -1;
  unsigned long long c[RT_N_COUNTERS];
  if (read_counters(D, c) != 0) return -1;
  out->paths = c[RT_CNT_PATHS];
  out->rays = c[RT_CNT_RAYS];
  out->node_visits = c[RT_CNT_NODES];
  out->leaf_visits = c[RT_CNT_LEAVES];
  out->shades = c[RT_CNT_SHADES];
  out->backgrounds = c[RT_CNT_BG];
  out->textured = c[RT_CNT_TEXTURED];
  return 0;
}

static float timed_slot_ms(Workspace &W, size_t slot) {
  if (hipEventSynchronize(W.ev1[slot]) != hipSuccess) return -1.0f;
  return event_ms(W.ev0[slot], W.ev1[slot]);
}

extern "C" f32 rt_last_kernel_ms(void) {
  Device &D = dev0();
  std::lock_guard<std::mutex> lock(D.mutex);
  if (!D.ready || D.ws.n_timed == 0) return -1.0f;
  DeviceGuard guard(D);
  return timed_slot_ms(D.ws, (D.ws.n_timed - 1) % RT_MAX_TIMED);
}

extern "C" void rt_kernel_timing_reset(void) {
  Device &D = dev0();
  std::lock_guard<std::mutex> lock(D.mutex);
  D.ws.n_timed = 0;
}

extern "C" f32 rt_kernel_timing_mean_ms(i32 *n_launches) {
  Device &D = dev0();
  std::lock_guard<std::mutex> lock(D.mutex);
  size_t n = D.ws.n_timed < RT_MAX_TIMED ? D.ws.n_timed : RT_MAX_TIMED;
  if (n_launches) *n_launches = (i32)n;
  if (!D.ready || n == 0) return -1.0f;
  DeviceGuard guard(D);
  double sum = 0.0;
  for (size_t i = 0; i < n; i++) {
    float ms = timed_slot_ms(D.ws, i);
    if (ms < 0.0f) return -1.0f;
    sum += ms;
  }
  return (float)(sum / (double)n);
}
```

### raytracing_c_amd/csrc/rt_tile.hip.h

```cpp
#ifndef RT_TILE_HIP_H
#define RT_TILE_HIP_H

typedef const RT_KView __attribute__((address_space(4))) *RT_KViewP;
template <bool VIEWS> struct CamSrc { typedef RT_KArgs type; };
template <> struct CamSrc<true> { typedef RT_KViewP type; };

__device__ __forceinline__ int take_queue_tile(const int lane, bool &queue_open) {
  RT_KArgs A = cold_args();
  uint32_t pos = 0;
  if (lane == 0) pos = atomicAdd(A->work_head, 1u);
  pos = (uint32_t)__builtin_amdgcn_readfirstlane((int)pos);
  const uint32_t *order = A->order;
  if (pos < (uint32_t)A->n_tiles) return order ? (int)order[pos] : (int)pos;
  queue_open = false;
  return -1;
}

__device__ __forceinline__ int join_open_tile(const int lane, const int wave_id, const int steal_tries, const uint32_t n_chunks_tile,
                                              uint32_t *lg = nullptr) {
  LGT0();
  int tile_idx = -1;
  RT_KArgs A = cold_args();
  const int n_tiles = A->n_tiles;
  const uint32_t *open_groups = A->open_groups, *tile_next = A->tile_next;
  const int n_groups = (n_tiles + 63) >> 6;
  const int g_rounds = (n_groups + 63) >> 6;
  const uint32_t hsh = ((uint32_t)wave_id * 2654435761u + (uint32_t)steal_tries * 40503u) >> 8;
  const int g_start = (int)(hsh % (uint32_t)g_rounds);
  for (int i = 0; i < g_rounds && tile_idx < 0; i++) {
    int r = g_start + i;
    if (r >= g_rounds) r -= g_rounds;
    int g = r * 64 + lane;
    uint32_t n_open = 0;
    if (g < n_groups) n_open = __hip_atomic_load(&open_groups[g], __ATOMIC_RELAXED, __HIP_MEMORY_SCOPE_AGENT);
    unsigned long long gm = __ballot(n_open != 0u);
    while (gm && tile_idx < 0) {
      int nth = (int)((hsh >> 6) % (uint32_t)__popcll(gm));
      unsigned long long m = gm;
      for (int k = 0; k < nth; k++) m &= m - 1ull;
      int gl = (int)__builtin_ctzll(m);
      gm &= ~(1ull << gl);
      int cand = (r * 64 + gl) * 64 + lane;
      uint32_t taken = 0xFFFFFFFFu;
      if (cand < n_tiles) taken = __hip_atomic_load(&tile_next[cand], __ATOMIC_RELAXED, __HIP_MEMORY_SCOPE_AGENT);
      unsigned long long open = __ballot(taken < n_chunks_tile);
      if (open) {
        const int n_open_tiles = (int)__popcll(open);
        int best = 0;
        uint32_t best_taken = 0xFFFFFFFFu;
#pragma unroll
        for (int c = 0; c < RT_JOIN_CHOICES; c++) {
          int nt = (int)(((hsh >> 12) * (uint32_t)(2 * c + 1) + (uint32_t)c * 7u) % (uint32_t)n_open_tiles);
          unsigned long long mm = open;
          for (int k = 0; k < nt; k++) mm &= mm - 1ull;
          const int pk_lane = (int)__builtin_ctzll(mm);
          const uint32_t tk = (uint32_t)__builtin_amdgcn_readlane((int)taken, pk_lane);
          if (tk < best_taken) { best_taken = tk; best = pk_lane; }
        }
        tile_idx = cand - lane + best;
      }
    }
  }
  LGT1(LG_CYC_JOIN);
  return tile_idx;
}

template <bool VIEWS>
__device__ __forceinline__ bool tile_origin(const int lane, const int tile_idx, const uint32_t n_chunks_tile, int &tile_x0, int &tile_y0,
                                            RT_KViewP &vrec) {
  RT_KArgs A = cold_args();
  int vt = tile_idx;
  if constexpr (VIEWS) {
    const int tu = __builtin_amdgcn_readfirstlane(tile_idx);
    const uint32_t view = (uint32_t)tu / (uint32_t)A->tiles_per_view;
    vt = tu - (int)view * A->tiles_per_view;
    vrec = (RT_KViewP)A->views + view;
  }
  const int lchunk = vt >> 4, sub = vt & 15;
  const int chunk = A->local_chunks[lchunk];
  const int chunks_x = A->chunks_x;
  tile_x0 = (chunk % chunks_x) * 32 + (sub & 3) * 8;
  tile_y0 = (chunk / chunks_x) * 32 + (sub >> 2) * 8;
  if (tile_x0 < A->width && tile_y0 < A->height) return true;
  if (lane == 0) {
    uint32_t old = atomicMax(&A->tile_next[tile_idx], n_chunks_tile);
    if (old < n_chunks_tile) atomicSub(&A->open_groups[tile_idx >> 6], 1u);
  }
  return false;
}
__device__ __forceinline__ bool tile_origin(const int lane, const int tile_idx, const uint32_t n_chunks_tile, int &tile_x0, int &tile_y0) {
  RT_KViewP no_view = nullptr;
  return tile_origin<false>(lane, tile_idx, n_chunks_tile, tile_x0, tile_y0, no_view);
}

template <class CAM>
__device__ __forceinline__ bool tile_pyramid(const CAM S, const float *nodes, float4 *smem, const int pyr_off, const int lane,
                                             const int tile_x0, const int tile_y0) {
  RT_KArgs A = cold_args();
  const float m = 0.05f;
  const float ux0 = ((float)tile_x0 - 0.5f - m) * 2.0f * A->inv_width - 1.0f;
  const float ux1 = ((float)tile_x0 + 7.5f + m) * 2.0f * A->inv_width - 1.0f;
  const float uy0 = ((float)tile_y0 - 0.5f - m) * 2.0f * A->inv_height - 1.0f;
  const float uy1 = ((float)tile_y0 + 7.5f + m) * 2.0f * A->inv_height - 1.0f;
  const float asp = A->aspect, fl = S->focal_length;
  rt_v3 c[4];
#pragma unroll
  for (int q = 0; q < 4; q++) {
    float cx = ((q == 1 || q == 2) ? ux1 : ux0) * asp, cy = -((q >= 2) ? uy1 : uy0), cz = -fl;
    c[q] = rt_v3_make(S->cam[0][0] * cx + S->cam[0][1] * cy + S->cam[0][2] * cz,
                      S->cam[1][0] * cx + S->cam[1][1] * cy + S->cam[1][2] * cz,
                      S->cam[2][0] * cx + S->cam[2][1] * cy + S->cam[2][2] * cz);
  }
  const rt_v3 o = rt_v3_make(S->cam[0][3], S->cam[1][3], S->cam[2][3]);
  rt_v3 pn[4];
#pragma unroll
  for (int q = 0; q < 4; q++) {
    rt_v3 n = rt_v3_cross(c[q], c[(q + 1) & 3]);
    if (rt_v3_dot(n, c[(q + 2) & 3]) > 0.0f) n = rt_v3_scale(n, -1.0f);
    pn[q] = n;
  }
  float *pyr = lds_at(smem, pyr_off);
  if (lane == 0) {
#pragma unroll
    for (int q = 0; q < 4; q++) { pyr[RT_PYR_PLANE + q * 4 + 0] = pn[q].x; pyr[RT_PYR_PLANE + q * 4 + 1] = pn[q].y; pyr[RT_PYR_PLANE + q * 4 + 2] = pn[q].z; }
    pyr[RT_PYR_ORIGIN] = o.x; pyr[RT_PYR_ORIGIN + 1] = o.y; pyr[RT_PYR_ORIGIN + 2] = o.z;
  }
  if (lane < RT_PYR_CACHE_WORDS) reinterpret_cast<uint32_t *>(pyr)[RT_PYR_LEAF_CACHE + lane] = 0u;
  bool may_hit = false;
  if (lane < 8) {
    const float *nb = nodes + lane;
    rt_v3 lo = rt_v3_make(nb[0] - o.x, nb[8] - o.y, nb[16] - o.z);
    rt_v3 hi = rt_v3_make(nb[24] - o.x, nb[32] - o.y, nb[40] - o.z);
    bool outside = child_box_empty(nb);
#pragma unroll
    for (int q = 0; q < 4; q++) {
      rt_v3 n = pn[q];
      float lox = n.x * lo.x, hix = n.x * hi.x, loy = n.y * lo.y, hiy = n.y * hi.y, loz = n.z * lo.z, hiz = n.z * hi.z;
      float nearest = fminf(lox, hix) + fminf(loy, hiy) + fminf(loz, hiz);
      float extent = fmaxf(fabsf(lox), fabsf(hix)) + fmaxf(fabsf(loy), fabsf(hiy)) + fmaxf(fabsf(loz), fabsf(hiz));
      float coarse = fabsf(n.x) * (fabsf(o.x) + fmaxf(fabsf(nb[0]), fabsf(nb[24]))) + fabsf(n.y) * (fabsf(o.y) + fmaxf(fabsf(nb[8]), fabsf(nb[32]))) +
                     fabsf(n.z) * (fabsf(o.z) + fmaxf(fabsf(nb[16]), fabsf(nb[40])));
      if (nearest > 1e-3f * extent + 1e-6f * coarse) outside = true;
    }
    may_hit = !outside;
  }
  return __ballot(may_hit) == 0ull;
}

#define RT_LL_MAX   32
#define RT_LL_ENTRY 0
#define RT_LL_NODE  RT_LL_MAX
#define RT_LL_GROUP 0x40000000u
static_assert(2 * RT_LL_MAX * 4 <= RT_LDS_PERM_LEVEL_BYTES && RT_LL_MAX <= 32, "the list is one row of the perm stack, `entered` one word");
__device__ __forceinline__ uint32_t *leafless_list(float4 *smem, const int pyr_off, const int levels) {
  return reinterpret_cast<uint32_t *>(lds_at(smem, pyr_off) - levels * (RT_LDS_PERM_LEVEL_BYTES / 4));
}
__device__ __forceinline__ int leafless_walk(float4 *smem, const float4 *lds_nodes, const int pyr_off, const int levels, const int n_nodes,
                                             const int leaf0, const float *leaves) {
  const float *pyr = lds_at(smem, pyr_off);
  uint32_t *list = leafless_list(smem, pyr_off, levels);
  int n_list = 1;
  for (int head = 0; head < n_list; head++) {
    const int nd = head ? __builtin_amdgcn_readfirstlane((int)list[RT_LL_NODE + head]) : 0;
    if (nd >= leaf0) continue;
    const uint32_t surv = 0xFFu & ~pyramid_cull_mask(lds_nodes, pyr, nd);
    if (lane_now() == 0) reinterpret_cast<uint32_t *>(lds_at(smem, pyr_off))[RT_PYR_NODE_CACHE + (nd & 31)] = ((uint32_t)(nd + 1) << 8) | (0xFFu & ~surv);
    if (surv) {
      const int ns = (int)__popc(surv);
      const bool groups = 8 * nd + 1 >= leaf0;
      if ((!groups && 8 * nd + 8 >= n_nodes) || ns > 4 || n_list + ns > RT_LL_MAX) return 0;
      if (groups) {
        for (uint32_t m = surv; m; m &= m - 1u) {
          const int g = 8 * nd + 1 + (int)__builtin_ctz(m) - leaf0;
          if ((uint32_t)g >= 0x800000u) return 0;
          uint32_t padding = 0u;
          const uint32_t cull = pyramid_cull_tris<true>(leaves, pyr, g, &padding);
          if (lane_now() == 0) reinterpret_cast<uint32_t *>(lds_at(smem, pyr_off))[RT_PYR_LEAF_CACHE + (g & 7)] = ((0x800000u | (uint32_t)g) << 8) | cull;
          if ((0xFFu & ~(cull | padding)) != 0u) return 0;
        }
      }
      const int k = lane_now();
      if (k < 8 && ((surv >> k) & 1u)) {
        const int at = n_list + (int)__popc(surv & ((1u << k) - 1u));
        list[RT_LL_ENTRY + at] = (uint32_t)(nd * RT_LDS_NODE_BYTES + k * 4) | ((uint32_t)head << 20) | (groups ? RT_LL_GROUP : 0u) | 0x80000000u;
        list[RT_LL_NODE + at] = (uint32_t)(8 * nd + 1 + k);
      }
      n_list += ns;
    }
  }
  return n_list;
}

struct TileUnits {
  uint32_t u_cur, u_end, grab;
  int  c_next, c_end;
  int  c_x0, c_y, c_pix0, c_s0;
  bool took_any;
};
__device__ __forceinline__ void tile_units_init(TileUnits &U, const bool queue_open) {
  U.c_next = U.c_end = U.c_x0 = U.c_y = U.c_pix0 = U.c_s0 = 0;
  U.u_cur = U.u_end = 0;
  U.grab = queue_open ? (uint32_t)cold_args()->grab_max : 1u;
  U.took_any = false;
}

__device__ __forceinline__ bool grab_units(const int lane, const int tile_idx, const uint32_t n_chunks_tile, uint32_t *tile_next,
                                           uint32_t *open_groups, const uint32_t gmax, TileUnits &U, const unsigned long long t_wave_start,
                                           unsigned long long &t_last_grab, uint32_t *lg = nullptr) {
  uint32_t u0 = 0;
  if (lane == 0) u0 = atomicAdd(&tile_next[tile_idx], U.grab);
  u0 = (uint32_t)__builtin_amdgcn_readfirstlane((int)u0);
  if (u0 >= n_chunks_tile) return false;
  U.u_cur = u0;
  U.u_end = u0 + U.grab < n_chunks_tile ? u0 + U.grab : n_chunks_tile;
  if (U.u_end == n_chunks_tile && lane == 0) atomicSub(&open_groups[tile_idx >> 6], 1u);
  if (t_wave_start) t_last_grab = __builtin_amdgcn_s_memrealtime();
  LG(LG_GRAB_X, 1);
  const uint32_t left = n_chunks_tile - U.u_end;
  U.grab = left >= 8u * gmax ? gmax : (left >= 8u && gmax >= 2u ? 2u : 1u);
  U.took_any = true;
  return true;
}

__device__ __forceinline__ void unit_decode(TileUnits &U, const int tile_x0, const int tile_y0, const int shift, const int unit_paths,
                                            const uint32_t n_sb, const int sample_first, const int width, const int height) {
  const uint32_t grp = U.u_cur >> 2, pair = U.u_cur & 3u;
  const uint32_t row = grp / n_sb, sb = grp - row * n_sb;
  U.c_x0 = tile_x0 + (int)pair * 2;
  U.c_y = tile_y0 + (int)row;
  U.c_pix0 = (int)row * 8 + (int)pair * 2;
  U.c_s0 = sample_first + (int)(sb << shift);
  U.c_next = 0;
  U.c_end = (U.c_y < height && U.c_x0 < width) ? unit_paths : 0;
}

struct NewPath { int x, y, sample, pix; };
__device__ __forceinline__ bool regen_paths(const int &phase, NewPath &np, const bool start_paths, TileUnits &U, bool &tile_open, const bool no_grab,
                                            const int lane, const int tile_idx, const uint32_t n_chunks_tile, const int tile_x0, const int tile_y0,
                                            const int shift, const int unit_paths, const unsigned long long t_wave_start,
                                            unsigned long long &t_last_grab, uint32_t &w_paths, uint32_t *lg = nullptr) {
  RT_KArgs A = cold_args();
  unsigned long long need = __ballot(phase == PH_NEED);
  bool got = false;
  const int width = A->width, sample_end = A->sample_end;
  LGM("regen_begin");
  while (need) {
    LG(LG_REGEN_X, 1);
    if (U.c_next >= U.c_end) {
      if (U.u_cur + 1u < U.u_end) {
        U.u_cur += 1u;
      } else if (no_grab || !grab_units(lane, tile_idx, n_chunks_tile, A->tile_next, A->open_groups, (uint32_t)A->grab_max, U, t_wave_start, t_last_grab LG_ARG)) {
        tile_open = false;
        break;
      }
      unit_decode(U, tile_x0, tile_y0, shift, unit_paths, (uint32_t)A->n_sample_blocks, A->sample_first, width, A->height);
      continue;
    }
    const int n_need = (int)__popcll(need);
    const int avail = U.c_end - U.c_next;
    const int take = n_need < avail ? n_need : avail;
    const int rank = lane_rank(need);
    bool valid = false;
    if (phase == PH_NEED && !got && rank < take) {
      const int k = U.c_next + rank;
      const int px = k >> shift;
      const int sm = U.c_s0 + (k & ((1 << shift) - 1));
      const int x = U.c_x0 + px;
      if (x < width && sm < sample_end) {
        valid = true;
        if (start_paths) { got = true; np.x = x; np.y = U.c_y; np.sample = sm; np.pix = U.c_pix0 + px; }
      }
    }
    w_paths += (uint32_t)__popcll(__ballot(valid));
    U.c_next += take;
    need = __ballot(phase == PH_NEED && !got);
  }
  LGM("regen_end");
  return got;
}

__device__ __forceinline__ void flush_tile(unsigned long long *acc, const int lane, const int tile_x0, const int tile_y0,
                                           unsigned long long *frame, const int tile_idx, const uint32_t n_rays) {
  const int x = tile_x0 + (lane & 7), y = tile_y0 + (lane >> 3);
  const unsigned long long r = acc[lane * 3 + 0], g = acc[lane * 3 + 1], b = acc[lane * 3 + 2];
  acc[lane * 3 + 0] = 0ull;
  acc[lane * 3 + 1] = 0ull;
  acc[lane * 3 + 2] = 0ull;
  RT_KArgs A = cold_args();
  const int width = A->width;
  if (x < width && y < A->height && (r | g | b) != 0ull) {
    unsigned long long *dst = frame + ((size_t)y * width + x) * 3;
    atomicAdd(dst + 0, r);
    atomicAdd(dst + 1, g);
    atomicAdd(dst + 2, b);
  }
  if (tile_idx >= 0) {
    uint32_t *tile_cost = A->tile_cost;
    if (tile_cost && lane == 0) atomicAdd(&tile_cost[tile_idx], n_rays);
  }
}

#endif
```

### raytracing_c_amd/csrc/rt_wavefront.hip

```cpp

#include "rt_dev.hip.h"

#define WF_NONE 0xFFFFFFFFu

struct WfOut {
  uint32_t chunk;
  int      pos;
};

template <int FIELDS>
__device__ __forceinline__ bool wf_append(uint32_t *data, uint32_t *cnt, uint32_t *alloc, WfOut &o, bool has,
                                          const uint32_t (&v)[FIELDS], uint32_t soft_chunks) {
  const unsigned long long m = __ballot(has);
  bool over = false;
  if (m == 0ull) return over;
  const int n = (int)__popcll(m);
  if (o.pos + n > WF_CHUNK) {
    const int lane = lane_now();
    if (o.chunk != WF_NONE && lane == 0) cnt[o.chunk] = (uint32_t)o.pos;
    uint32_t c = 0;
    if (lane == 0) c = atomicAdd(alloc, 1u);
    o.chunk = (uint32_t)__builtin_amdgcn_readfirstlane((int)c);
    o.pos = 0;
    over = o.chunk >= soft_chunks;
  }
  const int rank = lane_rank(m);
  if (has) {
    uint32_t *dst = data + (size_t)o.chunk * (FIELDS * WF_CHUNK) + (uint32_t)(o.pos + rank);
#pragma unroll
    for (int i = 0; i < FIELDS; i++) dst[i * WF_CHUNK] = v[i];
  }
  o.pos += n;
  return over;
}

__device__ __forceinline__ void wf_close(uint32_t *cnt, const WfOut &o) {
  if (o.chunk != WF_NONE && lane_now() == 0) cnt[o.chunk] = (uint32_t)o.pos;
}

__device__ __forceinline__ void wf_finish_consumer(uint32_t *ctl, int n_waves, int w_alloc, int w_head) {
  if (lane_now() == 0) {
    __builtin_amdgcn_fence(__ATOMIC_RELEASE, "agent");
    const uint32_t done = atomicAdd(&ctl[WF_DONE_WAVES * WF_CTL_STRIDE], 1u);
    if (done + 1u == (uint32_t)n_waves) {
      __hip_atomic_store(&ctl[w_alloc * WF_CTL_STRIDE], 0u, __ATOMIC_RELAXED, __HIP_MEMORY_SCOPE_AGENT);
      __hip_atomic_store(&ctl[w_head * WF_CTL_STRIDE], 0u, __ATOMIC_RELAXED, __HIP_MEMORY_SCOPE_AGENT);
      __hip_atomic_store(&ctl[WF_DONE_WAVES * WF_CTL_STRIDE], 0u, __ATOMIC_RELAXED, __HIP_MEMORY_SCOPE_AGENT);
    }
  }
}

template <int WAVES, bool LDSN, int MIN_WAVES_PER_SIMD, bool SHORT_DIV>
__global__ __launch_bounds__(WAVES * 64, MIN_WAVES_PER_SIMD) void rt_wf_camera_kernel(RT_KParams P) {
  extern __shared__ float4 smem[];
  const int lane = threadIdx.x & 63;
  const int wave = threadIdx.x >> 6;
  const int n_lds = LDSN ? P.n_lds_nodes : 0;
  const float4 *lds_nodes = smem;
  const WaveLds L = wave_lds(smem, n_lds, P.depth, wave);
  unsigned long long *acc = L.acc;
  const int acc_off = L.acc_off, pyr_off = L.pyr_off;

  if (LDSN) {
    lds_load_nodes<WAVES * 64>(smem, P.nodes, n_lds);
    __syncthreads();
  }

  acc_tile_clear(acc, lane);

  uint32_t w_paths = 0, w_rays = 0, w_nodes = 0, w_leaves = 0, w_bgs = 0;
  const int shift = P.chunk_shift;
  const int unit_paths = 2 << shift;
  const uint32_t n_chunks_tile = (uint32_t)P.n_chunks_tile;
  const int leaf_level = P.depth - 1;
  const int thresh = P.sched_thresh;
  const int pyr_nodes = LDSN ? P.pyr_nodes : 0;
  const int wave_id = (int)blockIdx.x * WAVES + wave;
  const TravWave W = {smem, lds_nodes, L.perm, n_lds, pyr_nodes, pyr_off, leaf_level, lane};

  bool queue_open = true, stopped = false;
  int  steal_tries = 0;
  WfOut out;
  out.chunk = WF_NONE;
  out.pos = WF_CHUNK;

  for (;;) {
    if (stopped) break;
    int tile_idx = queue_open ? take_queue_tile(lane, queue_open) : -1;
    if (tile_idx < 0) {
      if (steal_tries >= RT_STEAL_TRIES) break;
      steal_tries += 1;
      tile_idx = join_open_tile(lane, wave_id, steal_tries, n_chunks_tile);
      if (tile_idx < 0) break;
    }

    int tile_x0, tile_y0;
    if (!tile_origin(lane, tile_idx, n_chunks_tile, tile_x0, tile_y0)) continue;
    bool tile_root_miss = false;
    if (leaf_level >= 0) tile_root_miss = tile_pyramid(cold_args(), P.nodes, smem, pyr_off, lane, tile_x0, tile_y0);
    rt_v3 cam_o;
    {
      RT_KArgs A = cold_args();
      cam_o = rt_v3_make(A->cam[0][3], A->cam[1][3], A->cam[2][3]);
    }
    const uint32_t rays_before = w_rays;

    int   pix = 0, smp = 0;
    Ray3  ray;
    ray_setup(ray, cam_o, rt_v3_make(0, 0, 1));
    TravState T = RT_TRAV_IDLE;

    bool tile_open = true;
    TileUnits U;
    tile_units_init(U, queue_open);
    unsigned long long no_time = 0ull;

    for (;;) {
      {
        RT_KArgs A = cold_args();
        bool  done = false, start = false;
        rt_v3 radiance = rt_v3_make(0, 0, 0);
        if (T.phase == PH_MISS) {
          ShadeParams SP;
          shade_params(SP, A, false);
          radiance = background_lookup(SP, ray.d);
          done = true;
        }
        w_bgs += (uint32_t)__popcll(__ballot(done));
        {
          const uint32_t rec[WF_HIT0_FIELDS] = {(uint32_t)as_i(ray.d.x), (uint32_t)as_i(ray.d.y), (uint32_t)as_i(ray.d.z),
                                                (uint32_t)as_i(T.hit.t), (uint32_t)T.hit.tri, (uint32_t)as_i(T.hit.u), (uint32_t)as_i(T.hit.v),
                                                (uint32_t)(tile_x0 + (pix & 7)) | ((uint32_t)(tile_y0 + (pix >> 3)) << 16), (uint32_t)smp};
          const bool is_hit = T.phase == PH_HIT;
          if (wf_append<WF_HIT0_FIELDS>(A->wf_hit0, A->wf_cnt_hit0, A->wf_ctl + WF_HIT0_ALLOC * WF_CTL_STRIDE, out, is_hit, rec,
                                        (uint32_t)A->wf_soft_chunks)) {
            if (!stopped && lane == 0) __hip_atomic_store(A->wf_ctl + WF_STOPPED * WF_CTL_STRIDE, 1u, __ATOMIC_RELAXED, __HIP_MEMORY_SCOPE_AGENT);
            stopped = true;
            queue_open = false;
          }
          if (is_hit) T.phase = PH_NEED;
        }
        if (done) {
          tile_add_sample(smem, acc_off, pix, radiance);
          T.phase = PH_NEED;
        }

        rt_v3 dir = ray.d;
        if (tile_open) {
          NewPath np = {0, 0, 0, 0};
          const bool got = regen_paths(T.phase, np, A->max_bounces > 0, U, tile_open, stopped, lane, tile_idx, n_chunks_tile, tile_x0, tile_y0,
                                       shift, unit_paths, 0ull, no_time, w_paths);
          if (got) {
            pix = np.pix;
            smp = np.sample;
            PrimaryParams PP;
            primary_params(PP, A, A);
            rt_v3 org;
            primary_ray(PP, np.x, np.y, np.sample, org, dir);
            start = true;
          }
        }
        bool skip_root = false;
        if (start) {
          ray_setup<SHORT_DIV>(ray, cam_o, dir);
          trav_start(T, leaf_level, P.last_row_offset);
          skip_root = tile_root_miss && ray.fast;
          if (skip_root) T.phase = PH_MISS;
        }
        w_rays += (uint32_t)__popcll(__ballot(start));
        w_nodes += (uint32_t)__popcll(__ballot(skip_root));
      }

      const int n_trav0 = (int)__popcll(__ballot(T.phase == PH_NODE || T.phase == PH_LEAF));
      if (n_trav0 == 0) {
        if (__any(T.phase == PH_MISS)) continue;
        if (!tile_open) break;
        continue;
      }

      traversal_blocks<LDSN, SHORT_DIV, true>(P, W, ray, true, T, thresh, n_trav0, w_nodes, w_leaves);
    }

    if (U.took_any) {
      flush_tile(acc, lane, tile_x0, tile_y0, cold_args()->accum, tile_idx, w_rays - rays_before);
      steal_tries = 0;
    }
  }
  RT_KArgs A = cold_args();
  wf_close(A->wf_cnt_hit0, out);
  unsigned long long *counters = A->counters;
  if (lane == 0) {
    atomicAdd(counters + RT_CNT_PATHS, (unsigned long long)w_paths);
    atomicAdd(counters + RT_CNT_RAYS, (unsigned long long)w_rays);
    atomicAdd(counters + RT_CNT_NODES, (unsigned long long)w_nodes);
    atomicAdd(counters + RT_CNT_LEAVES, (unsigned long long)w_leaves);
    atomicAdd(counters + RT_CNT_BG, (unsigned long long)w_bgs);
  }
}

template <int WAVES, bool LDSN, int MIN_WAVES_PER_SIMD, bool SHORT_DIV>
__global__ __launch_bounds__(WAVES * 64, MIN_WAVES_PER_SIMD) void rt_wf_trace_kernel(RT_KParams P) {
  extern __shared__ float4 smem[];
  const int lane = threadIdx.x & 63;
  const int wave = threadIdx.x >> 6;
  const int n_lds = LDSN ? P.n_lds_nodes : 0;
  const float4 *lds_nodes = smem;
  const WaveLds L = wave_lds(smem, n_lds, P.depth, wave);
  unsigned long long *acc = L.acc;
  const int acc_off = L.acc_off;

  if (LDSN) {
    lds_load_nodes<WAVES * 64>(smem, P.nodes, n_lds);
    __syncthreads();
  }
  acc_tile_clear(acc, lane);
  uint32_t acc_key = 0xFFFFFFFFu;

  uint32_t w_rays = 0, w_nodes = 0, w_leaves = 0, w_bgs = 0;
  const int leaf_level = P.depth - 1;
  const TravWave W = {smem, lds_nodes, L.perm, n_lds, 0, 0, leaf_level, lane};
  const int thresh = P.sched_thresh;
  const int qi = (P.wf_bounce - 1) & 1;
  const int w_in_alloc = WF_RAY0_ALLOC + 2 * qi, w_in_head = WF_RAY0_HEAD + 2 * qi;

  uint32_t n_in;
  {
    RT_KArgs A = cold_args();
    n_in = (uint32_t)__builtin_amdgcn_readfirstlane((int)A->wf_ctl[w_in_alloc * WF_CTL_STRIDE]);
  }
  bool input_open = true;
  uint32_t rc = 0;
  int rpos = 0, rcnt = 0;
  WfOut out;
  out.chunk = WF_NONE;
  out.pos = WF_CHUNK;

  uint32_t ray_idx = 0;
  Ray3  ray;
  ray_setup(ray, rt_v3_make(0, 0, 0), rt_v3_make(0, 0, 1));
  TravState T = RT_TRAV_IDLE;

  for (;;) {
    {
      RT_KArgs A = cold_args();
      const uint32_t *rq = A->wf_ray[qi];
      const unsigned long long mMiss = __ballot(T.phase == PH_MISS);
      if (mMiss) {
        rt_v3 radiance = rt_v3_make(0, 0, 0);
        uint32_t pixel = 0;
        if (T.phase == PH_MISS) {
          const uint32_t *rr = rq + (size_t)(ray_idx >> 8) * (WF_RAY_FIELDS * WF_CHUNK) + (ray_idx & 255u);
          const rt_v3 tint = rt_v3_make(as_f((int)rr[6 * WF_CHUNK]), as_f((int)rr[7 * WF_CHUNK]), as_f((int)rr[8 * WF_CHUNK]));
          const rt_v3 emis = rt_v3_make(as_f((int)rr[9 * WF_CHUNK]), as_f((int)rr[10 * WF_CHUNK]), as_f((int)rr[11 * WF_CHUNK]));
          pixel = rr[13 * WF_CHUNK];
          ShadeParams SP;
          shade_params(SP, A, false);
          const rt_v3 bg = background_lookup(SP, ray.d);
          radiance = rt_v3_mul_add(bg, tint, emis);
        }
        unsigned long long *frame = A->accum;
        if (frame) {
          const uint32_t key = ((pixel >> 19) << 13) | ((pixel & 0xFFFFu) >> 3);
          const uint32_t k0 = (uint32_t)__builtin_amdgcn_readlane((int)key, (int)__builtin_ctzll(mMiss));
          if (k0 != acc_key) {
            if (acc_key != 0xFFFFFFFFu)
              flush_tile(reinterpret_cast<unsigned long long *>(lds_at(smem, acc_off)), lane_now(), (int)(acc_key & 8191u) * 8,
                         (int)(acc_key >> 13) * 8, frame, -1, 0u);
            acc_key = k0;
          }
          if (T.phase == PH_MISS) {
            if (key == acc_key) {
              tile_add_sample(smem, acc_off, (int)(((pixel >> 16) & 7u) * 8u + (pixel & 7u)), radiance);
            } else {
              const unsigned long long qr = accum_quantize_dev(radiance.x), qg = accum_quantize_dev(radiance.y), qb = accum_quantize_dev(radiance.z);
              unsigned long long *dst = frame + ((size_t)(pixel >> 16) * A->width + (pixel & 0xFFFFu)) * 3;
              if (qr) atomicAdd(dst + 0, qr);
              if (qg) atomicAdd(dst + 1, qg);
              if (qb) atomicAdd(dst + 2, qb);
            }
          }
        }
      }
      w_bgs += (uint32_t)__popcll(__ballot(T.phase == PH_MISS));
      {
        const uint32_t rec[WF_HIT_FIELDS] = {ray_idx, (uint32_t)as_i(T.hit.t), (uint32_t)T.hit.tri, (uint32_t)as_i(T.hit.u), (uint32_t)as_i(T.hit.v)};
        wf_append<WF_HIT_FIELDS>(A->wf_hit, A->wf_cnt_hit, A->wf_ctl + WF_HIT_ALLOC * WF_CTL_STRIDE, out, T.phase == PH_HIT, rec, 0xFFFFFFFFu);
      }
      if (T.phase == PH_MISS || T.phase == PH_HIT) T.phase = PH_NEED;

      bool start = false;
      rt_v3 org = ray.o, dir = ray.d;
      if (input_open) {
        unsigned long long need = __ballot(T.phase == PH_NEED);
        while (need) {
          if (rpos >= rcnt) {
            uint32_t c = 0;
            if (lane == 0) c = atomicAdd(A->wf_ctl + w_in_head * WF_CTL_STRIDE, 1u);
            c = (uint32_t)__builtin_amdgcn_readfirstlane((int)c);
            if (c >= n_in) { input_open = false; break; }
            rc = c;
            rcnt = (int)__builtin_amdgcn_readfirstlane((int)A->wf_cnt_ray[qi][c]);
            rpos = 0;
            continue;
          }
// ... 197 lines not shown
```

### raytracing_c_amd/ctypes_abi.py

```python
import ctypes as C

import numpy as np

isize = C.c_ssize_t
f32 = C.c_float


class Vec2(C.Structure):
    _fields_ = [("x", f32), ("y", f32)]


class Vec3(C.Structure):
    _fields_ = [("x", f32), ("y", f32), ("z", f32)]


class Matrix_4x4(C.Structure):
    _fields_ = [("rows", (f32 * 4) * 4)]


class Byte_Slice(C.Structure):
    _fields_ = [("data", C.c_void_p), ("len", isize)]


class Image(C.Structure):
# ... 66 lines not shown
    _fields_ = [("position", Vec3), ("direction", Vec3)]


class Hit(C.Structure):
    _fields_ = [("distance", f32), ("normal", Vec3), ("normal_geo", Vec3), ("point", Vec3),
                ("tangent", Vec3), ("bitangent", Vec3), ("tex_coords", Vec2), ("shader", Shader)]


class Rendering_Context(C.Structure):
    _fields_ = [("image", Image), ("scene", C.POINTER(Scene)), ("samples", isize), ("max_bounces", isize),
                ("n_threads", C.c_int32), ("_current_chunk", C.c_int32)]


class PBR_Shader_Data(C.Structure):
    _fields_ = [("base_color", Vec3), ("emission", Vec3),
                ("roughness", f32), ("metalness", f32), ("normal_map_strength", f32),
                ("sheen", f32), ("sheen_tint", f32), ("anisotropic_strength", f32),
                ("texture_albedo", C.POINTER(Image)), ("texture_normal", C.POINTER(Image)),
                ("texture_metal_roughness", C.POINTER(Image)), ("texture_emission", C.POINTER(Image))]


class RT_Counters(C.Structure):
    _fields_ = [(n, C.c_uint64) for n in
                ("paths", "rays", "node_visits", "leaf_visits", "shades", "backgrounds", "textured")]


class RT_Frame_Timing(C.Structure):
    _fields_ = [(n, C.c_float) for n in
                ("stamp_ms", "upload_ms", "enqueue_ms", "gpu_prep_ms", "gpu_path_ms", "gpu_resolve_ms", "gpu_copy_ms", "total_ms",
                 "verify_ms", "gather_ms")] + [("n_devices", C.c_int32), ("slowest_device", C.c_int32)]


class RT_Render_Params(C.Structure):
    _fields_ = [("width", C.c_int32), ("height", C.c_int32), ("samples", C.c_int32), ("max_bounces", C.c_int32),
                ("seed", C.c_uint32), ("rank", C.c_int32), ("world", C.c_int32), ("slab", C.c_int32),
                ("flags", C.c_int32), ("sample_first", C.c_int32), ("sample_count", C.c_int32)]


class RT_View(C.Structure):
    _fields_ = [("camera", Camera), ("seed", C.c_uint32)]


class RT_Ray_Hit(C.Structure):
    _fields_ = [("t", f32), ("triangle", C.c_int32), ("u", f32), ("v", f32)]


class RT_Device_Hit(C.Structure):
    _fields_ = [("distance", f32), ("normal", Vec3), ("normal_geo", Vec3), ("point", Vec3),
                ("tangent", Vec3), ("bitangent", Vec3), ("tex_coords", Vec2),
                ("triangle", C.c_int32), ("material", C.c_int32), ("pad", C.c_int32 * 2)]


class RT_Query_Counters(C.Structure):
    _fields_ = [(n, C.c_uint64) for n in ("rays", "hits", "node_visits", "leaf_visits")]


class RT_Features(C.Structure):
    _fields_ = [(n, C.POINTER(f32)) for n in ("coverage", "albedo", "normal", "position")]


RT_FEATURE_CHANNELS = 10
RT_MOTION_CHANNELS = 3


class RT_Guided_Params(C.Structure):
    _fields_ = [("iterations", C.c_int32), ("sigma_color", f32), ("sigma_normal", f32), ("sigma_position", f32),
                ("demodulate", C.c_int32)]


assert C.sizeof(RT_Guided_Params) == 20


class RT_Temporal_Params(C.Structure):
    _fields_ = [("alpha", f32), ("max_history", C.c_int32), ("normal_tolerance", f32), ("plane_tolerance", f32),
                ("demodulate", C.c_int32)]


class RT_History_Planes(C.Structure):
    _fields_ = [(n, C.POINTER(f32)) for n in ("color", "length", "coverage", "normal", "position")]


assert C.sizeof(RT_Temporal_Params) == 20
RT_TEMPORAL_HISTORY_PER_PIXEL = 48


class RT_Variance_Params(C.Structure):
    _fields_ = [("sigma_normal", f32), ("sigma_position", f32)]


assert C.sizeof(RT_Variance_Params) == 8
RT_TEMPORAL_MOMENTS_PER_PIXEL = 16


class RT_Upsample_Params(C.Structure):
    _fields_ = [("sigma_normal", f32), ("sigma_position", f32), ("demodulate", C.c_int32), ("guide_samples", C.c_int32)]


assert C.sizeof(RT_Upsample_Params) == 16
RT_UPSAMPLE_WORK_PER_LOW_PIXEL = 48


class RT_Adaptive_Params(C.Structure):
    _fields_ = [("min_samples", C.c_int32), ("max_samples", C.c_int32), ("threshold", f32), ("reserved", C.c_int32)]


assert C.sizeof(RT_Adaptive_Params) == 16


RAY_HIT_DTYPE = np.dtype([("t", "<f4"), ("triangle", "<i4"), ("u", "<f4"), ("v", "<f4")])
_HIT_HEAD = [("distance", "<f4"), ("normal", "<f4", (3,)), ("normal_geo", "<f4", (3,)), ("point", "<f4", (3,)),
             ("tangent", "<f4", (3,)), ("bitangent", "<f4", (3,)), ("tex_coords", "<f4", (2,))]
DEVICE_HIT_DTYPE = np.dtype(_HIT_HEAD + [("triangle", "<i4"), ("material", "<i4"), ("pad", "<i4", (2,))])
HIT_DTYPE = np.dtype(_HIT_HEAD + [("shader_data", "<u8"), ("shader_proc", "<u8")])
assert RAY_HIT_DTYPE.itemsize == C.sizeof(RT_Ray_Hit) == 16
assert DEVICE_HIT_DTYPE.itemsize == C.sizeof(RT_Device_Hit) == 88
assert HIT_DTYPE.itemsize == C.sizeof(Hit) == 88
RT_QUERY_MAX_RAYS = 1 << 30
RT_QUERY_SLICE = 1 << 20

assert C.sizeof(BVH_Node) == 192
assert C.sizeof(Triangle) == 112
assert C.sizeof(Triangle_AOS) == 112
assert C.sizeof(Hit) == 88
assert C.sizeof(PBR_Shader_Data) == 80

TRIANGLE_DTYPE = np.dtype([("positions", "<f4", (3, 3)), ("normals", "<f4", (3, 3)), ("tex_coords", "<f4", (3, 2)),
                           ("shader_data", "<u8"), ("shader_proc", "<u8")])
assert TRIANGLE_DTYPE.itemsize == 112

EXPORTED_SYMBOLS = [
    "render_thread_proc", "rendering_context_is_finished", "rendering_context_finish", "lightmap_bake", "render",
    "denoise_image",
    "scene_init", "scene_init_sah", "scene_init_gpu", "rt_scene_alloc", "rt_scene_free", "scene_load_bytes", "scene_save_bytes", "scene_file_size",
    "rt_scene_slot_map", "scene_refit", "scene_refit_gpu",
    "disney_shader_proc", "debug_shader_proc", "sample_background",
    "rt_last_error", "rt_clear_error", "rt_init", "rt_set_seed", "rt_get_seed",
    "rt_set_devices", "rt_device_count", "rt_math_contract",
    "rt_scene_verify", "rt_scene_touch", "rt_scene_set_static", "rt_get_frame_timing",
    "rt_scene_upload", "rt_scene_release", "rt_scene_invalidate", "rt_scene_device_bytes", "rt_set_camera",
    "rt_device_scene_keep_geometry", "rt_scene_keep_geometry", "rt_scene_has_kept_geometry",
    "rt_chunk_count", "rt_chunk_owner", "rt_local_chunk_count", "rt_max_local_chunk_count", "rt_local_chunk_list", "rt_render_accumulate", "rt_resolve", "rt_untile",
    "rt_denoise", "rt_render_frame", "rt_frame_begin", "rt_frame_end", "rt_render_views", "rt_render_accumulate_views",
    "rt_query_closest", "rt_query_occluded", "rt_scene_hits", "rt_scene_closest", "rt_scene_occluded", "rt_get_query_counters",
    "rt_render_accumulate_features", "rt_resolve_features", "rt_render_features",
    "rt_render_accumulate_features_motion", "rt_resolve_motion", "rt_render_features_motion",
    "rt_guided_work_bytes", "rt_guided_denoise", "rt_guided_denoise_host", "rt_render_denoised",
    "rt_temporal_history_bytes", "rt_temporal_accumulate", "rt_temporal_accumulate_host", "rt_history_create", "rt_history_reset",
    "rt_history_destroy", "rt_history_set_motion", "rt_render_temporal",
    "rt_temporal_moments_bytes", "rt_temporal_accumulate_moments", "rt_temporal_accumulate_moments_host",
    "rt_temporal_accumulate_motion", "rt_temporal_accumulate_motion_host",
    "rt_guided_variance_work_bytes", "rt_guided_denoise_variance", "rt_guided_denoise_variance_host", "rt_render_svgf",
    "rt_guided_upsample_work_bytes", "rt_guided_upsample", "rt_guided_upsample_host", "rt_render_upsampled",
    "rt_render_accumulate_chunks", "rt_adaptive_merge", "rt_resolve_adaptive", "rt_render_adaptive",
    "rt_get_counters", "rt_get_skipped_root_visits", "rt_get_leafless_paths", "rt_get_triangleless_paths", "rt_get_fused_root_visits", "rt_get_shade_taps_form", "rt_materials_share_taps", "rt_last_kernel_ms", "rt_kernel_timing_reset", "rt_kernel_timing_mean_ms",
]

DIAG_ONLY_SYMBOLS = [
    "rt_diag_set_tokens", "rt_diag_multi_fault", "rt_set_pipeline", "rt_get_pipeline", "rt_set_wavefront_capacity", "rt_get_wave_times", "rt_get_ledger",
    "rt_diag_device_bytes_live", "rt_diag_release_staging", "rt_diag_cached_scene",
    "rt_test_math", "rt_test_rcp_sweep", "rt_test_srgb_sweep", "rt_test_env_sweep", "rt_test_quantize_sweep", "rt_test_encode_sweep", "rt_test_group_sum", "rt_test_sky_add_group", "rt_test_node_order", "rt_test_trace", "rt_test_trace_stream",
    "rt_test_tile_order", "rt_test_texture", "rt_test_shade", "rt_test_shade_hit", "rt_test_feature_hit", "rt_test_brdf", "rt_test_background", "rt_test_primary_ray",
]
```

### raytracing_c_amd/native.py

```python
import ctypes as C
import os

from . import ctypes_abi as abi

_HERE = os.path.dirname(os.path.abspath(__file__))
LIB_PATH = os.environ.get("RT_LIB_PATH") or os.path.join(_HERE, "librt_hip.so")
DIAG_PATH = os.path.join(_HERE, "librt_hip_diag.so")


class NativeLibraryMissing(RuntimeError):
    pass


def _preload_hip_runtime():
    import importlib.util
    import sys
    if os.environ.get("RT_HIP_RUNTIME", "torch") != "torch":
        return
    if "torch" in sys.modules:
        return
    try:
        spec = importlib.util.find_spec("torch")
    except (ImportError, ValueError):
        spec = None
# ... 17 lines not shown
    def _load(self):
        if self._dll is not None:
            return self._dll
        if not os.path.exists(self._path):
            raise NativeLibraryMissing(
                f"{self._path} not found: build it with `make -C raytracing_c_amd/csrc{' diag' if self._diag else ''}` "
                "(or __graft_entry__.build()); there is no CPU fallback for the render path")
        _preload_hip_runtime()
        dll = C.CDLL(self._path)
        _declare(dll)
        if self._diag or hasattr(dll, "rt_test_math"):
            _declare_diag(dll)
        if self._diag and os.path.realpath(self._path) != os.path.realpath(LIB_PATH):
            dll.rt_diag_set_tokens(symbol_address("disney_shader_proc"), symbol_address("debug_shader_proc"),
                                   symbol_address("sample_background"))
        self._dll = dll
        return dll

    def __getattr__(self, name):
        return getattr(self._load(), name)


def _declare(d):
    P = C.POINTER
    vp = C.c_void_p
    d.rt_last_error.restype = C.c_char_p
    d.rt_clear_error.restype = None
    d.rt_init.argtypes = [C.c_int]
    d.rt_set_seed.argtypes = [C.c_uint32]
    d.rt_set_seed.restype = None
    d.rt_get_seed.restype = C.c_uint32
    d.scene_init.argtypes = [P(abi.Scene), abi.Triangle_Slice, abi.Allocator]
    d.scene_init.restype = None
    d.scene_init_sah.argtypes = [P(abi.Scene), abi.Triangle_Slice, abi.Allocator]
    d.scene_init_sah.restype = None
    d.scene_init_gpu.argtypes = [P(abi.Scene), abi.Triangle_Slice, abi.Allocator]
    if hasattr(d, "scene_refit"):
        d.rt_scene_slot_map.argtypes = [P(abi.Scene), abi.Triangle_Slice, vp]
        d.rt_scene_slot_map.restype = C.c_ssize_t
        d.scene_refit.argtypes = [P(abi.Scene), abi.Triangle_Slice, vp]
        d.scene_refit_gpu.argtypes = [P(abi.Scene), abi.Triangle_Slice, vp]
    d.rt_scene_alloc.argtypes = [P(abi.Scene), abi.isize, abi.Allocator]
    d.rt_scene_alloc.restype = C.c_bool
    d.rt_scene_free.argtypes = [P(abi.Scene)]
    d.rt_scene_free.restype = None
    d.scene_load_bytes.argtypes = [abi.Byte_Slice, P(abi.Scene)]
    d.scene_load_bytes.restype = C.c_bool
    d.scene_save_bytes.argtypes = [P(abi.Scene), vp, C.c_ssize_t]
    d.scene_save_bytes.restype = C.c_ssize_t
    d.scene_file_size.argtypes = [P(abi.Scene)]
    d.scene_file_size.restype = C.c_ssize_t
    d.rt_scene_upload.argtypes = [P(abi.Scene)]
    d.rt_scene_upload.restype = vp
    d.rt_scene_release.argtypes = [vp]
    d.rt_scene_release.restype = None
    d.rt_scene_invalidate.argtypes = [P(abi.Scene)]
    d.rt_scene_invalidate.restype = None
    d.rt_scene_device_bytes.argtypes = [vp]
    d.rt_scene_device_bytes.restype = C.c_int64
    d.rt_set_camera.argtypes = [vp, P(abi.Camera)]
    d.rt_chunk_count.argtypes = [C.c_int32, C.c_int32]
    d.rt_local_chunk_count.argtypes = [C.c_int32] * 4
    d.rt_chunk_owner.argtypes = [C.c_int32] * 4
    d.rt_max_local_chunk_count.argtypes = [C.c_int32] * 3
    d.rt_local_chunk_list.argtypes = [C.c_int32] * 4 + [P(C.c_int32), C.c_int32]
    d.rt_render_accumulate.argtypes = [vp, P(abi.RT_Render_Params), vp, vp]
    d.rt_resolve.argtypes = [P(abi.RT_Render_Params), vp, vp, vp, vp, vp]
    d.rt_untile.argtypes = [C.c_int32, C.c_int32, C.c_int32, vp, vp, vp]
    d.rt_render_frame.argtypes = [P(abi.Scene), P(abi.Image), abi.isize, abi.isize, vp, vp]
    if hasattr(d, "rt_frame_begin"):
        d.rt_frame_begin.argtypes = [P(abi.Scene), P(abi.Image), abi.isize, abi.isize]
        d.rt_frame_end.argtypes = [C.c_int]
    if hasattr(d, "rt_render_views"):
        d.rt_render_views.argtypes = [P(abi.Scene), C.c_int32, P(abi.RT_View), P(abi.Image), abi.isize, abi.isize, vp, vp]
        d.rt_render_accumulate_views.argtypes = [vp, P(abi.RT_Render_Params), C.c_int32, P(abi.RT_View), vp, vp]
    if hasattr(d, "rt_query_closest"):
        d.rt_query_closest.argtypes = [vp, C.c_int64, vp, vp, vp, vp, vp]
        d.rt_query_occluded.argtypes = [vp, C.c_int64, vp, vp, vp, vp]
        d.rt_scene_hits.argtypes = [P(abi.Scene), C.c_int64, vp, vp, vp]
        d.rt_scene_closest.argtypes = [P(abi.Scene), C.c_int64, vp, vp, vp]
        d.rt_scene_occluded.argtypes = [P(abi.Scene), C.c_int64, vp, vp, vp]
        d.rt_get_query_counters.argtypes = [P(abi.RT_Query_Counters)]
    if hasattr(d, "rt_render_features"):
        d.rt_render_accumulate_features.argtypes = [vp, P(abi.RT_Render_Params), vp, vp]
        d.rt_resolve_features.argtypes = [P(abi.RT_Render_Params), vp, vp, vp, vp, vp, vp]
        d.rt_render_features.argtypes = [P(abi.Scene), C.c_int32, C.c_int32, abi.isize, abi.isize, P(abi.RT_Features), vp]
    if hasattr(d, "rt_guided_denoise"):
        d.rt_guided_work_bytes.argtypes = [C.c_int32, C.c_int32]
        d.rt_guided_work_bytes.restype = C.c_int64
        d.rt_guided_denoise.argtypes = [C.c_int32, C.c_int32, P(abi.RT_Guided_Params)] + [vp] * 9
        d.rt_guided_denoise_host.argtypes = [C.c_int32, C.c_int32, P(abi.RT_Guided_Params), vp, P(abi.RT_Features), vp, vp]
        d.rt_render_denoised.argtypes = [P(abi.Scene), P(abi.Image), abi.isize, abi.isize, P(abi.RT_Guided_Params), vp, vp]
    if hasattr(d, "rt_temporal_accumulate"):
        d.rt_temporal_history_bytes.argtypes = [C.c_int32, C.c_int32]
        d.rt_temporal_history_bytes.restype = C.c_int64
        d.rt_temporal_accumulate.argtypes = [C.c_int32, C.c_int32, P(abi.RT_Temporal_Params), P(abi.Camera), P(abi.Camera)] + [vp] * 11
        d.rt_temporal_accumulate_host.argtypes = [C.c_int32, C.c_int32, P(abi.RT_Temporal_Params), P(abi.Camera), P(abi.Camera), vp,
                                                  P(abi.RT_Features), P(abi.RT_History_Planes), P(abi.RT_History_Planes), vp, vp, vp]
        d.rt_history_create.argtypes = [C.c_int32, C.c_int32]
        d.rt_history_create.restype = vp
        d.rt_history_reset.argtypes = [vp]
        d.rt_history_destroy.argtypes = [vp]
        d.rt_history_destroy.restype = None
        d.rt_render_temporal.argtypes = [P(abi.Scene), P(abi.Image), abi.isize, abi.isize, vp, P(abi.RT_Temporal_Params),
                                         P(abi.RT_Guided_Params), vp, vp, vp]
    if hasattr(d, "rt_render_svgf"):
        d.rt_temporal_moments_bytes.argtypes = [C.c_int32, C.c_int32]
        d.rt_temporal_moments_bytes.restype = C.c_int64
        d.rt_temporal_accumulate_moments.argtypes = ([C.c_int32, C.c_int32, P(abi.RT_Temporal_Params), P(abi.Camera), P(abi.Camera)]
                                                     + [vp] * 10 + [P(abi.RT_Variance_Params)] + [vp] * 4)
        d.rt_temporal_accumulate_moments_host.argtypes = [C.c_int32, C.c_int32, P(abi.RT_Temporal_Params), P(abi.Camera), P(abi.Camera),
                                                          vp, P(abi.RT_Features), P(abi.RT_History_Planes), P(abi.RT_History_Planes),
                                                          vp, vp, vp, P(abi.RT_Variance_Params), vp, vp, vp]
        d.rt_guided_variance_work_bytes.argtypes = [C.c_int32, C.c_int32]
        d.rt_guided_variance_work_bytes.restype = C.c_int64
        d.rt_guided_denoise_variance.argtypes = [C.c_int32, C.c_int32, P(abi.RT_Guided_Params)] + [vp] * 11
        d.rt_guided_denoise_variance_host.argtypes = [C.c_int32, C.c_int32, P(abi.RT_Guided_Params), vp, P(abi.RT_Features), vp, vp, vp,
                                                      vp]
        d.rt_render_svgf.argtypes = [P(abi.Scene), P(abi.Image), abi.isize, abi.isize, vp, P(abi.RT_Temporal_Params),
                                     P(abi.RT_Variance_Params), P(abi.RT_Guided_Params), vp, vp, vp, vp]
    if hasattr(d, "rt_render_upsampled"):
        d.rt_guided_upsample_work_bytes.argtypes = [C.c_int32, C.c_int32]
        d.rt_guided_upsample_work_bytes.restype = C.c_int64
        d.rt_guided_upsample.argtypes = [C.c_int32, C.c_int32, P(abi.RT_Upsample_Params)] + [vp] * 13
        d.rt_guided_upsample_host.argtypes = [C.c_int32, C.c_int32, P(abi.RT_Upsample_Params), vp, P(abi.RT_Features),
                                              P(abi.RT_Features), vp, vp]
        d.rt_render_upsampled.argtypes = [P(abi.Scene), P(abi.Image), abi.isize, abi.isize, P(abi.RT_Upsample_Params),
                                          P(abi.RT_Guided_Params), vp, vp, vp]
    if hasattr(d, "rt_render_adaptive"):
        d.rt_render_accumulate_chunks.argtypes = [vp, P(abi.RT_Render_Params), C.c_int32, vp, vp, vp]
        d.rt_adaptive_merge.argtypes = [C.c_int32] * 4 + [vp] * 5
        d.rt_resolve_adaptive.argtypes = [C.c_int32, C.c_int32] + [vp] * 6
        d.rt_render_adaptive.argtypes = [P(abi.Scene), P(abi.Image), P(abi.RT_Adaptive_Params), abi.isize, vp, vp, vp]
    if hasattr(d, "rt_scene_keep_geometry"):
        d.rt_device_scene_keep_geometry.argtypes = [vp, vp]
        d.rt_scene_keep_geometry.argtypes = [P(abi.Scene)]
        d.rt_scene_has_kept_geometry.argtypes = [P(abi.Scene)]
        d.rt_render_accumulate_features_motion.argtypes = [vp, P(abi.RT_Render_Params), vp, vp, vp]
        d.rt_resolve_motion.argtypes = [P(abi.RT_Render_Params), vp, vp, vp]
        d.rt_render_features_motion.argtypes = [P(abi.Scene), C.c_int32, C.c_int32, abi.isize, abi.isize, P(abi.RT_Features), vp, vp, vp]
        d.rt_temporal_accumulate_motion.argtypes = ([C.c_int32, C.c_int32, P(abi.RT_Temporal_Params), P(abi.Camera), P(abi.Camera)]
                                                    + [vp] * 10 + [P(abi.RT_Variance_Params)] + [vp] * 5)
        d.rt_temporal_accumulate_motion_host.argtypes = [C.c_int32, C.c_int32, P(abi.RT_Temporal_Params), P(abi.Camera), P(abi.Camera),
                                                         vp, P(abi.RT_Features), P(abi.RT_History_Planes), P(abi.RT_History_Planes),
                                                         vp, vp, vp, P(abi.RT_Variance_Params), vp, vp, vp, vp]
        d.rt_history_set_motion.argtypes = [vp, C.c_int]
    d.rt_get_counters.argtypes = [P(abi.RT_Counters)]
    if hasattr(d, "rt_get_skipped_root_visits"):
        d.rt_get_skipped_root_visits.argtypes = [P(C.c_uint64)]
    if hasattr(d, "rt_get_leafless_paths"):
        d.rt_get_leafless_paths.argtypes = [P(C.c_uint64)]
    if hasattr(d, "rt_get_triangleless_paths"):
        d.rt_get_triangleless_paths.argtypes = [P(C.c_uint64)]
    if hasattr(d, "rt_get_fused_root_visits"):
        d.rt_get_fused_root_visits.argtypes = [P(C.c_uint64)]
    if hasattr(d, "rt_get_shade_taps_form"):
        d.rt_get_shade_taps_form.argtypes = []
        d.rt_materials_share_taps.argtypes = [vp, C.c_int32]
    d.rt_math_contract.restype = C.c_int
    d.rt_last_kernel_ms.restype = C.c_float
    d.rt_kernel_timing_reset.restype = None
    d.rt_kernel_timing_mean_ms.argtypes = [P(C.c_int32)]
    d.rt_kernel_timing_mean_ms.restype = C.c_float
    d.rt_set_devices.argtypes = [C.c_int32, C.c_int32]
    d.rt_device_count.restype = C.c_int32
    d.rt_scene_verify.argtypes = [P(abi.Scene)]
    d.rt_scene_touch.argtypes = [P(abi.Scene), vp, C.c_size_t]
    d.rt_scene_set_static.argtypes = [P(abi.Scene), C.c_int32]
    d.rt_scene_set_static.restype = None
    d.rt_get_frame_timing.argtypes = [P(abi.RT_Frame_Timing)]
    d.render_thread_proc.argtypes = [P(abi.Rendering_Context)]
    d.render_thread_proc.restype = None
    d.rendering_context_is_finished.argtypes = [P(abi.Rendering_Context)]
    d.rendering_context_is_finished.restype = C.c_bool
    d.rendering_context_finish.argtypes = [P(abi.Rendering_Context)]
    d.rendering_context_finish.restype = None
    d.render.argtypes = [P(abi.Scene), P(abi.Image), abi.isize, abi.isize]
    d.lightmap_bake.argtypes = [P(abi.Image), P(abi.Scene), abi.isize]
    d.lightmap_bake.restype = None
    d.denoise_image.argtypes = [P(abi.Image), P(abi.Image), abi.isize]
    d.denoise_image.restype = None
    d.rt_denoise.argtypes = [C.c_int32, C.c_int32, vp, vp, vp]


def _declare_diag(d):
    vp = C.c_void_p
    d.rt_test_math.argtypes = [C.c_int32, C.c_int32, vp, vp, vp]
    d.rt_test_rcp_sweep.argtypes = [vp]
    d.rt_test_srgb_sweep.argtypes = [vp]
    d.rt_test_env_sweep.argtypes = [C.c_int32, C.c_uint32, vp]
    d.rt_test_quantize_sweep.argtypes = [vp]
    d.rt_test_encode_sweep.argtypes = [vp]
    d.rt_test_group_sum.argtypes = [C.c_int32, C.c_int32, vp, vp, vp]
    d.rt_test_sky_add_group.argtypes = []
    d.rt_test_node_order.argtypes = [C.c_int32, vp, vp, vp]
    d.rt_test_trace.argtypes = [vp, C.c_int32, vp, vp, vp, vp]
    d.rt_test_texture.argtypes = [vp, C.c_int32, C.c_int32, vp, vp]
    d.rt_test_shade.argtypes = [vp, C.c_int32, C.c_int32] + [vp] * 7
    d.rt_test_shade_hit.argtypes = [vp, C.c_int32, C.c_int32, C.c_int32] + [vp] * 8
    d.rt_test_feature_hit.argtypes = [vp, C.c_int32] + [vp] * 5
    d.rt_test_brdf.argtypes = [C.c_int32] + [vp] * 6
    d.rt_test_background.argtypes = [vp, C.c_int32, C.c_int32, vp, vp]
    d.rt_test_primary_ray.argtypes = [C.POINTER(abi.Camera), C.c_int32, C.c_int32, C.c_int32, vp, vp]
    d.rt_test_trace_stream.argtypes = [vp, C.c_int32, vp, vp, C.c_int32, C.c_int32, vp, vp, vp, vp]
    d.rt_test_tile_order.argtypes = [C.c_int32, vp, vp]
    d.rt_set_pipeline.argtypes = [C.c_int32]
    d.rt_get_pipeline.restype = C.c_int32
    d.rt_set_wavefront_capacity.argtypes = [C.c_int64]
    d.rt_set_wavefront_capacity.restype = None
    d.rt_get_wave_times.argtypes = [vp, C.c_int32]
    d.rt_get_ledger.argtypes = [vp, C.c_int32]
    d.rt_diag_device_bytes_live.argtypes = []
    d.rt_diag_device_bytes_live.restype = C.c_int64
    d.rt_diag_release_staging.argtypes = []
    d.rt_diag_cached_scene.argtypes = [C.POINTER(abi.Scene)]
    d.rt_diag_cached_scene.restype = vp
    d.rt_diag_multi_fault.argtypes = [C.c_int32, C.c_int32]
    d.rt_diag_multi_fault.restype = None
    d.rt_diag_set_tokens.argtypes = [vp, vp, vp]
    d.rt_diag_set_tokens.restype = None


lib = _Lazy(LIB_PATH)
diag = _Lazy(DIAG_PATH, diag=True)


def symbol_address(name):
    return C.cast(getattr(lib, name), C.c_void_p).value


def last_error(which=None):
    return ((which or lib).rt_last_error() or b"").decode("utf-8", "replace")
```

### raytracing_c_amd/tile_classes.py

```python
import numpy as np

F = np.float32


def lds_nodes(n_nodes, depth, wg_waves=16):
    per_wave = max(depth, 1) * 256 + 1536
    room = (160 * 1024 - 64 - wg_waves * per_wave) // 208
    return min(n_nodes, max(room, 0))


def tile_pyramids(cam_rows, focal_length, width, height):
    cam = np.asarray(cam_rows, F).reshape(-1, 4)[:3]
    ty, tx = (height + 7) // 8, (width + 7) // 8
    inv_w, inv_h, asp = F(1.0) / F(width), F(1.0) / F(height), F(width) / F(height)
    m = F(0.05)
    x0 = (np.arange(tx, dtype=F) * F(8))[None, :]
    y0 = (np.arange(ty, dtype=F) * F(8))[:, None]
    ux0 = (x0 - F(0.5) - m) * F(2.0) * inv_w - F(1.0)
    ux1 = (x0 + F(7.5) + m) * F(2.0) * inv_w - F(1.0)
    uy0 = (y0 - F(0.5) - m) * F(2.0) * inv_h - F(1.0)
    uy1 = (y0 + F(7.5) + m) * F(2.0) * inv_h - F(1.0)
    c = np.zeros((ty, tx, 4, 3), F)
    for q in range(4):
        cx = np.broadcast_to((ux1 if q in (1, 2) else ux0) * asp, (ty, tx))
        cy = np.broadcast_to(-(uy1 if q >= 2 else uy0), (ty, tx))
        cz = F(-focal_length)
        for i in range(3):
            c[:, :, q, i] = cam[i, 0] * cx + cam[i, 1] * cy + cam[i, 2] * cz
    pn = np.zeros((ty, tx, 4, 3), F)
    for q in range(4):
        n = np.cross(c[:, :, q], c[:, :, (q + 1) & 3]).astype(F)
        flip = np.sum(n * c[:, :, (q + 2) & 3], axis=-1) > 0
        n[flip] = -n[flip]
        pn[:, :, q] = n
    return pn, cam[:, 3].copy()


def cull_masks(nodes, node_idx, pn, origin, margin=1e-3):
    nb = nodes[node_idx]
    mn, mx = nb[:, 0:3, :], nb[:, 3:6, :]
    o = origin.astype(F)[None, :, None]
    empty = np.all(nb == 0, axis=1)
    nrm = pn[:, :, :, None]
    lo = nrm * (mn - o)[:, None]
    hi = nrm * (mx - o)[:, None]
    nearest = np.minimum(lo, hi).sum(axis=2, dtype=F)
    extent = np.maximum(np.abs(lo), np.abs(hi)).sum(axis=2, dtype=F)
    coarse = (np.abs(nrm) * (np.abs(o)[:, None] + np.maximum(np.abs(mn), np.abs(mx))[:, None])).sum(axis=2, dtype=F)
    with np.errstate(invalid="ignore"):
        outside = nearest > F(margin) * extent + F(1e-6) * coarse
    return empty | outside.any(axis=1)


def cull_tris(soa, group, pn, origin, margin=1e-3, zero_culled=True):
    soa = np.asarray(soa, F)
    n_groups = soa.shape[1] // 8
    inside = np.asarray(group) < n_groups
    slots = np.where(inside, group, 0)[:, None] * 8 + np.arange(8)[None, :]
    v = soa[:, slots] * inside[None, :, None].astype(F)
    a = np.stack([v[0], v[3], v[6]], axis=1)
    e1 = np.stack([v[1], v[4], v[7]], axis=1) - a
    e2 = np.stack([v[2], v[5], v[8]], axis=1) - a
    zero = np.all(v == 0, axis=0)
    o = origin.astype(F)[None, None, :, None]
    nrm = pn[:, :, :, None]
    with np.errstate(invalid="ignore", over="ignore"):
        band = F(2.5e-4) * (np.abs((nrm * e1[:, None]).sum(axis=2, dtype=F)) + np.abs((nrm * e2[:, None]).sum(axis=2, dtype=F)))
        outside = np.ones(band.shape, bool)
        for vert in (a, a + e1, a + e2):
            vert = vert[:, None]
            p = nrm * (vert - o)
            val = p.sum(axis=2, dtype=F)
            extent = np.abs(p).sum(axis=2, dtype=F)
            coarse = (np.abs(nrm) * (np.abs(o) + np.abs(vert))).sum(axis=2, dtype=F)
            outside &= val - band > F(margin) * extent + F(1e-6) * coarse
    culled = outside.any(axis=1)
    return culled | zero if zero_culled else culled


def _cull_chunked(nodes, node, pn, origin, margin, chunk=1 << 17):
    out = np.empty((len(node), 8), bool)
    for a in range(0, len(node), chunk):
        out[a:a + chunk] = cull_masks(nodes, node[a:a + chunk], pn[a:a + chunk], origin, margin)
    return out


def classify_tiles(nodes, depth, cam_rows, focal_length, width, height, margin=1e-3, give_up=64, tris=None, zero_culled=True):
    nodes = np.asarray(nodes, F).reshape(-1, 6, 8)
    pn, origin = tile_pyramids(cam_rows, focal_length, width, height)
    ty, tx = pn.shape[:2]
    n_tiles = ty * tx
    pn = pn.reshape(n_tiles, 4, 3)
    leaf_level = depth - 1
    reached_leaf = np.zeros(n_tiles, bool)
    n_listed = np.zeros(n_tiles, np.int64)
    max_surv = np.zeros(n_tiles, np.int64)
    max_node = np.zeros(n_tiles, np.int64)
    root_miss = np.zeros(n_tiles, bool)
    n_groups = np.zeros(n_tiles, np.int64)
    has_tri = np.zeros(n_tiles, bool)
    leaf0 = (8 ** max(depth, 0) - 1) // 7
    if leaf_level < 0 or len(nodes) == 0:
        reached_leaf[:] = True
    else:
        tile = np.arange(n_tiles)
        node = np.zeros(n_tiles, np.int64)
        for level in range(leaf_level + 1):
            if len(tile) == 0:
                break
            surv = ~_cull_chunked(nodes, node, pn[tile], origin, margin)
            ns = surv.sum(axis=1)
            np.add.at(n_listed, tile, 1)
            np.maximum.at(max_surv, tile, ns)
            np.maximum.at(max_node, tile, node)
            if level == 0:
                root_miss = ns == 0
            if level == leaf_level:
                reached_leaf[tile[ns > 0]] = True
                if tris is not None:
                    pi, k = np.nonzero(surv)
                    np.add.at(n_groups, tile[pi], 1)
                    group = 8 * node[pi] + 1 + k - leaf0
                    for a in range(0, len(pi), 1 << 15):
                        b = slice(a, a + (1 << 15))
                        kept = ~cull_tris(tris, group[b], pn[tile[pi[b]]], origin, margin, zero_culled)
                        has_tri[tile[pi[b]][kept.any(axis=1)]] = True
                break
            pi, k = np.nonzero(surv)
            tile, node = tile[pi], 8 * node[pi] + 1 + k
            reached_leaf[n_listed + np.bincount(tile, minlength=n_tiles) > give_up] = True
            keep = ~reached_leaf[tile]
            tile, node = tile[keep], node[keep]
    shape = (ty, tx)
    out = dict(root_miss=root_miss.reshape(shape), leafless=(~reached_leaf).reshape(shape), n_listed=n_listed.reshape(shape),
               max_surv=max_surv.reshape(shape), max_node=max_node.reshape(shape))
    if tris is not None:
        out.update(triangleless=((n_groups > 0) & ~has_tri).reshape(shape), n_groups=n_groups.reshape(shape),
                   n_entries=(n_listed - 1 + n_groups).reshape(shape))
    return out


def classify_scene(hs, width, height, margin=1e-3, triangles=False, zero_culled=True):
    cam = hs.scene.camera
    rows = [[cam.view_matrix.rows[i][j] for j in range(4)] for i in range(4)]
    return classify_tiles(hs.nodes_array(), hs.depth, rows, cam.focal_length, width, height, margin,
                          tris=hs.soa_array() if triangles else None, zero_culled=zero_culled)
```

Baseline: 24480 Mray/s.

## Cull triangles per pixel pair in mixed tiles to route clear pairs down the sky path

When a tile's pyramid walk reaches leaf groups with live triangles, it now builds frusta for each 2x1 pixel pair and checks whether those triangles can be culled for every pair (deep walk, on by default at 64 or more samples). Pairs that touch no triangle are recorded in an LDS bitmask, and unit decoding reorders work so clear pairs go first through the cheap sky path. The goal is to skip BVH traversal for primary rays in pairs that provably miss all geometry. The cost is a heavier per-tile walk with per-lane triangle tests, plus extra readlane and ballot logic in unit decoding.

```diff
diff --git a/include/rt_hip.h b/include/rt_hip.h
--- a/include/rt_hip.h
+++ b/include/rt_hip.h
@@ -264,6 +264,7 @@
 extern int rt_get_skipped_root_visits(u64 *out);
 extern int rt_get_leafless_paths(u64 *out);
 extern int rt_get_triangleless_paths(u64 *out);
+extern int rt_get_clear_pair_paths(u64 *out);
 extern int rt_get_fused_root_visits(u64 *out);
 extern int rt_get_shade_taps_form(void);
 extern int rt_materials_share_taps(f32 const *mats, i32 n_materials);
diff --git a/raytracing_c_amd/csrc/rt_dev.hip.h b/raytracing_c_amd/csrc/rt_dev.hip.h
--- a/raytracing_c_amd/csrc/rt_dev.hip.h
+++ b/raytracing_c_amd/csrc/rt_dev.hip.h
@@ -1159,6 +1159,7 @@
 #define RT_PYR_ORIGIN     16
 #define RT_PYR_ROOT_POP   19
 #define RT_PYR_ROOT_FUSED 20
+#define RT_PYR_CLEAR      21
 #define RT_PYR_LEAF_CACHE 24
 #define RT_PYR_NODE_CACHE 32
 #define RT_PYR_CACHE_WORDS 40
diff --git a/raytracing_c_amd/csrc/rt_device.h b/raytracing_c_amd/csrc/rt_device.h
--- a/raytracing_c_amd/csrc/rt_device.h
+++ b/raytracing_c_amd/csrc/rt_device.h
@@ -30,6 +30,7 @@
   RT_CNT_LEAFLESS = 136,
   RT_CNT_FUSED_ROOT,
   RT_CNT_TRIANGLELESS,
+  RT_CNT_CLEAR_PAIRS,
   RT_N_COUNTERS
 };
 #define RT_CNT_LEDGER_SLOTS (RT_CNT_LEAFLESS - RT_CNT_LEDGER)
@@ -69,7 +70,8 @@
   int32_t chunks_x, n_chunks;
   int32_t rank, world, n_local_chunks;
   int32_t shared_taps;
-  int32_t unused_pad[2];
+  int32_t deep_walk;
+  int32_t unused_pad;
   int32_t sched_thresh;
   int32_t n_lds_nodes;
   unsigned long long *accum;
diff --git a/raytracing_c_amd/csrc/rt_kernels.hip b/raytracing_c_amd/csrc/rt_kernels.hip
--- a/raytracing_c_amd/csrc/rt_kernels.hip
+++ b/raytracing_c_amd/csrc/rt_kernels.hip
@@ -99,7 +99,13 @@
     int n_list = 0;
     int ll_levels = leaf_level, ll_nodes = pyr_nodes, ll_leaf0 = P.last_row_offset;
     asm volatile("" : "+s"(ll_levels), "+s"(ll_nodes), "+s"(ll_leaf0));
-    if (ll_levels >= 1 && ll_nodes > 0 && !tile_root_miss) n_list = leafless_walk(smem, lds_nodes, pyr_off, ll_levels, ll_nodes, ll_leaf0, cold_args()->leaves);
+    uint32_t *clear_word = reinterpret_cast<uint32_t *>(lds_at(smem, pyr_off)) + RT_PYR_CLEAR;
+    if (lane_now() == 0) *clear_word = 0u;
+    if (ll_levels >= 1 && ll_nodes > 0 && !tile_root_miss) {
+      typename CamSrc<VIEWS>::type S;
+      if constexpr (VIEWS) S = vrec; else S = cold_args();
+      n_list = leafless_walk(smem, lds_nodes, pyr_off, ll_levels, ll_nodes, ll_leaf0, cold_args()->leaves, cold_args()->deep_walk != 0, S, tile_x0, tile_y0);
+    }
     const uint32_t rays_before = w_rays;
     LG(LG_TILE_X, 1);
     LGM("tile_end");
@@ -131,7 +137,7 @@
       uint32_t *tile_next = A->tile_next, *open_groups = A->open_groups;
       uint32_t n_sky = 0;
       const uint32_t *list = leafless_list(smem, pyr_off, ll_levels);
-      const uint32_t list_entry = (n_list > 1 && lane_now() < n_list) ? list[RT_LL_ENTRY + (lane_now() & 31)] : 0u;
+      const uint32_t list_entry = lane_now() == 63 ? *clear_word : ((n_list > 1 && lane_now() < n_list) ? list[RT_LL_ENTRY + (lane_now() & 31)] : 0u);
       for (;;) {
         if (U.c_next >= U.c_end) {
           if (U.u_cur + 1u < U.u_end) {
@@ -150,7 +156,8 @@
             U.grab = left >= 8u * gmax ? gmax : (left >= 8u && gmax >= 2u ? 2u : 1u);
             U.took_any = true;
           }
-          unit_decode(U, tile_x0, tile_y0, shift, unit_paths, n_sb, sample_first, width, height);
+          const uint32_t clear = (uint32_t)__builtin_amdgcn_readlane((int)list_entry, 63);
+          if (!unit_decode(U, tile_x0, tile_y0, shift, unit_paths, n_sb, sample_first, width, height, clear) && clear != 0u) break;
           continue;
         }
 #ifndef RT_SKY_PATHS
@@ -223,8 +230,10 @@
         LGT1(LG_CYC_SKY);
         LGM("sky_end");
       }
-      if (n_sky != 0u && lane == 0) atomicAdd(cold_args()->counters + (tile_root_miss ? RT_CNT_SKIPPED_ROOT : RT_CNT_LEAFLESS), (unsigned long long)n_sky);
-      if (n_sky != 0u && (__ballot((list_entry & RT_LL_GROUP) != 0u) & ~1ull) != 0ull && lane == 0)
+      const bool mixed = (uint32_t)__builtin_amdgcn_readlane((int)list_entry, 63) != 0u;
+      if (n_sky != 0u && lane == 0)
+        atomicAdd(cold_args()->counters + (tile_root_miss ? RT_CNT_SKIPPED_ROOT : (mixed ? RT_CNT_CLEAR_PAIRS : RT_CNT_LEAFLESS)), (unsigned long long)n_sky);
+      if (n_sky != 0u && !mixed && (__ballot((list_entry & RT_LL_GROUP) != 0u) & 0xFFFFFFFEull) != 0ull && lane == 0)
         atomicAdd(cold_args()->counters + RT_CNT_TRIANGLELESS, (unsigned long long)n_sky);
     }
 
@@ -334,7 +343,7 @@
         if (tile_open) {
           NewPath np = {0, 0, 0, 0};
           const bool got = regen_paths(T.phase, np, SP.max_bounces > 0, U, tile_open, false, lane, tile_idx, n_chunks_tile, tile_x0, tile_y0,
-                                       shift, unit_paths, t_wave_start, t_last_grab, w_paths LG_ARG);
+                                       shift, unit_paths, t_wave_start, t_last_grab, w_paths, clear_word LG_ARG);
           if (!tile_open) LGD0((int)__popcll(__ballot(T.phase != PH_NEED || got)) + n_parked);
           const int gx = np.x, gy = np.y, gs = np.sample, width = A->width;
 #ifdef RT_LEDGER
diff --git a/raytracing_c_amd/csrc/rt_launch.cpp b/raytracing_c_amd/csrc/rt_launch.cpp
--- a/raytracing_c_amd/csrc/rt_launch.cpp
+++ b/raytracing_c_amd/csrc/rt_launch.cpp
@@ -267,6 +267,11 @@
     if (v == 1 || v == 2 || v == 4) K.grab_max = v;
   }
   K.pyr_nodes = knob_int("RT_PYRAMID", 1) ? K.n_lds_nodes : 0;
+  K.deep_walk = n_samples >= 64 ? 1 : 0;
+  {
+    int v = knob_int("RT_DEEP_WALK", -1);
+    if (v == 0 || v == 1) K.deep_walk = v;
+  }
   float cam_max = 0.0f;
   for (int v = 0; v < nv; v++)
     for (int i = 0; i < 3; i++)
@@ -476,6 +481,8 @@
 
 extern "C" int rt_get_triangleless_paths(u64 *out) { return get_counter("rt_get_triangleless_paths", RT_CNT_TRIANGLELESS, out); }
 
+extern "C" int rt_get_clear_pair_paths(u64 *out) { return get_counter("rt_get_clear_pair_paths", RT_CNT_CLEAR_PAIRS, out); }
+
 extern "C" int rt_get_fused_root_visits(u64 *out) { return get_counter("rt_get_fused_root_visits", RT_CNT_FUSED_ROOT, out); }
 
 extern "C" int rt_get_shade_taps_form(void) { return g_taps_form.load(); }
diff --git a/raytracing_c_amd/csrc/rt_tile.hip.h b/raytracing_c_amd/csrc/rt_tile.hip.h
--- a/raytracing_c_amd/csrc/rt_tile.hip.h
+++ b/raytracing_c_amd/csrc/rt_tile.hip.h
@@ -155,11 +155,72 @@
 __device__ __forceinline__ uint32_t *leafless_list(float4 *smem, const int pyr_off, const int levels) {
   return reinterpret_cast<uint32_t *>(lds_at(smem, pyr_off) - levels * (RT_LDS_PERM_LEVEL_BYTES / 4));
 }
+template <class CAM>
+__device__ __forceinline__ void pair_planes(const CAM S, const int tile_x0, const int tile_y0, rt_v3 pn[4]) {
+  RT_KArgs A = cold_args();
+  const int p = lane_now() & 31;
+  const float m = 0.05f;
+  const float x = (float)(tile_x0 + 2 * (p & 3)), y = (float)(tile_y0 + (p >> 2));
+  const float ux0 = (x - 0.5f - m) * 2.0f * A->inv_width - 1.0f;
+  const float ux1 = (x + 1.5f + m) * 2.0f * A->inv_width - 1.0f;
+  const float uy0 = (y - 0.5f - m) * 2.0f * A->inv_height - 1.0f;
+  const float uy1 = (y + 0.5f + m) * 2.0f * A->inv_height - 1.0f;
+  const float asp = A->aspect, fl = S->focal_length;
+  rt_v3 c[4];
+#pragma unroll
+  for (int q = 0; q < 4; q++) {
+    float cx = ((q == 1 || q == 2) ? ux1 : ux0) * asp, cy = -((q >= 2) ? uy1 : uy0), cz = -fl;
+    c[q] = rt_v3_make(S->cam[0][0] * cx + S->cam[0][1] * cy + S->cam[0][2] * cz,
+                      S->cam[1][0] * cx + S->cam[1][1] * cy + S->cam[1][2] * cz,
+                      S->cam[2][0] * cx + S->cam[2][1] * cy + S->cam[2][2] * cz);
+  }
+#pragma unroll
+  for (int q = 0; q < 4; q++) {
+    rt_v3 n = rt_v3_cross(c[q], c[(q + 1) & 3]);
+    if (rt_v3_dot(n, c[(q + 2) & 3]) > 0.0f) n = rt_v3_scale(n, -1.0f);
+    pn[q] = n;
+  }
+}
+__device__ __forceinline__ bool pair_culls_tris(const rt_v3 pn[4], const float *pyr, const float *leaves, const int g, uint32_t live) {
+  const float ox = pyr[RT_PYR_ORIGIN], oy = pyr[RT_PYR_ORIGIN + 1], oz = pyr[RT_PYR_ORIGIN + 2];
+  cfloat *lb = as_scalar_ptr(leaves) + (size_t)g * 72;
+  bool all = true;
+  while (live) {
+    cfloat *tb = lb + (int)__builtin_ctz(live);
+    live &= live - 1u;
+    const float ax = tb[0], e1x = tb[8], e2x = tb[16], ay = tb[24], e1y = tb[32], e2y = tb[40], az = tb[48], e1z = tb[56], e2z = tb[64];
+    bool culled = false;
+#pragma unroll
+    for (int q = 0; q < 4; q++) {
+      const float nx = pn[q].x, ny = pn[q].y, nz = pn[q].z;
+      const float band = 2.5f * RT_EPS * (fabsf(nx * e1x + ny * e1y + nz * e1z) + fabsf(nx * e2x + ny * e2y + nz * e2z));
+      bool outside = true;
+#pragma unroll
+      for (int v = 0; v < 3; v++) {
+        const float vx = v == 0 ? ax : (v == 1 ? ax + e1x : ax + e2x);
+        const float vy = v == 0 ? ay : (v == 1 ? ay + e1y : ay + e2y);
+        const float vz = v == 0 ? az : (v == 1 ? az + e1z : az + e2z);
+        const float px = nx * (vx - ox), py = ny * (vy - oy), pz = nz * (vz - oz);
+        const float val = px + py + pz;
+        const float extent = fabsf(px) + fabsf(py) + fabsf(pz);
+        const float coarse = fabsf(nx) * (fabsf(ox) + fabsf(vx)) + fabsf(ny) * (fabsf(oy) + fabsf(vy)) + fabsf(nz) * (fabsf(oz) + fabsf(vz));
+        outside = outside && (val - band > 1e-3f * extent + 1e-6f * coarse);
+      }
+      culled = culled || outside;
+    }
+    all = all && culled;
+  }
+  return all;
+}
+
+template <class CAM>
 __device__ __forceinline__ int leafless_walk(float4 *smem, const float4 *lds_nodes, const int pyr_off, const int levels, const int n_nodes,
-                                             const int leaf0, const float *leaves) {
+                                             const int leaf0, const float *leaves, const bool deep, const CAM S, const int tile_x0,
+                                             const int tile_y0) {
   const float *pyr = lds_at(smem, pyr_off);
   uint32_t *list = leafless_list(smem, pyr_off, levels);
   int n_list = 1;
+  bool mixed = false, clear = true;
   for (int head = 0; head < n_list; head++) {
     const int nd = head ? __builtin_amdgcn_readfirstlane((int)list[RT_LL_NODE + head]) : 0;
     if (nd >= leaf0) continue;
@@ -176,7 +237,15 @@
           uint32_t padding = 0u;
           const uint32_t cull = pyramid_cull_tris<true>(leaves, pyr, g, &padding);
           if (lane_now() == 0) reinterpret_cast<uint32_t *>(lds_at(smem, pyr_off))[RT_PYR_LEAF_CACHE + (g & 7)] = ((0x800000u | (uint32_t)g) << 8) | cull;
-          if ((0xFFu & ~(cull | padding)) != 0u) return 0;
+          const uint32_t live = 0xFFu & ~(cull | padding);
+          if (live != 0u) {
+            if (!deep) return 0;
+            rt_v3 ppn[4];
+            pair_planes(S, tile_x0, tile_y0, ppn);
+            clear = clear && pair_culls_tris(ppn, pyr, leaves, g, live);
+            mixed = true;
+            if ((uint32_t)__ballot(clear) == 0u) return 0;
+          }
         }
       }
       const int k = lane_now();
@@ -187,6 +256,11 @@
       }
       n_list += ns;
     }
+  }
+  if (mixed) {
+    const uint32_t mask = (uint32_t)__ballot(clear);
+    if (mask == 0u) return 0;
+    if (lane_now() == 0) reinterpret_cast<uint32_t *>(lds_at(smem, pyr_off))[RT_PYR_CLEAR] = mask;
   }
   return n_list;
 }
@@ -222,23 +296,42 @@
   return true;
 }
 
-__device__ __forceinline__ void unit_decode(TileUnits &U, const int tile_x0, const int tile_y0, const int shift, const int unit_paths,
-                                            const uint32_t n_sb, const int sample_first, const int width, const int height) {
-  const uint32_t grp = U.u_cur >> 2, pair = U.u_cur & 3u;
-  const uint32_t row = grp / n_sb, sb = grp - row * n_sb;
+__device__ __forceinline__ bool unit_decode(TileUnits &U, const int tile_x0, const int tile_y0, const int shift, const int unit_paths,
+                                            const uint32_t n_sb, const int sample_first, const int width, const int height,
+                                            const uint32_t clear = 0u) {
+  uint32_t row, sb, pair;
+  bool is_clear = false;
+  if (clear != 0u) {
+    const uint32_t n_clear = (uint32_t)__popc(clear) * n_sb;
+    is_clear = U.u_cur < n_clear;
+    const uint32_t v = is_clear ? U.u_cur : U.u_cur - n_clear, m = is_clear ? clear : ~clear;
+    const uint32_t j = v / n_sb;
+    sb = v - j * n_sb;
+    const int l = lane_now();
+    const bool mine = l < 32 && ((m >> (l & 31)) & 1u) != 0u && (uint32_t)__popc(m & ((1u << (l & 31)) - 1u)) == j;
+    const uint32_t p = (uint32_t)__builtin_ctzll(__ballot(mine) | (1ull << 63));
+    row = (p >> 2) & 7u;
+    pair = p & 3u;
+  } else {
+    const uint32_t grp = U.u_cur >> 2;
+    pair = U.u_cur & 3u;
+    row = grp / n_sb;
+    sb = grp - row * n_sb;
+  }
   U.c_x0 = tile_x0 + (int)pair * 2;
   U.c_y = tile_y0 + (int)row;
   U.c_pix0 = (int)row * 8 + (int)pair * 2;
   U.c_s0 = sample_first + (int)(sb << shift);
   U.c_next = 0;
   U.c_end = (U.c_y < height && U.c_x0 < width) ? unit_paths : 0;
+  return is_clear;
 }
 
 struct NewPath { int x, y, sample, pix; };
 __device__ __forceinline__ bool regen_paths(const int &phase, NewPath &np, const bool start_paths, TileUnits &U, bool &tile_open, const bool no_grab,
                                             const int lane, const int tile_idx, const uint32_t n_chunks_tile, const int tile_x0, const int tile_y0,
                                             const int shift, const int unit_paths, const unsigned long long t_wave_start,
-                                            unsigned long long &t_last_grab, uint32_t &w_paths, uint32_t *lg = nullptr) {
+                                            unsigned long long &t_last_grab, uint32_t &w_paths, const uint32_t *clear_word, uint32_t *lg = nullptr) {
   RT_KArgs A = cold_args();
   unsigned long long need = __ballot(phase == PH_NEED);
   bool got = false;
@@ -247,13 +340,16 @@
   while (need) {
     LG(LG_REGEN_X, 1);
     if (U.c_next >= U.c_end) {
+      uint32_t clear = 0u;
+      if (clear_word) clear = *clear_word;
       if (U.u_cur + 1u < U.u_end) {
         U.u_cur += 1u;
       } else if (no_grab || !grab_units(lane, tile_idx, n_chunks_tile, A->tile_next, A->open_groups, (uint32_t)A->grab_max, U, t_wave_start, t_last_grab LG_ARG)) {
         tile_open = false;
         break;
       }
-      unit_decode(U, tile_x0, tile_y0, shift, unit_paths, (uint32_t)A->n_sample_blocks, A->sample_first, width, A->height);
+      unit_decode(U, tile_x0, tile_y0, shift, unit_paths, (uint32_t)A->n_sample_blocks, A->sample_first, width, A->height,
+                  clear_word ? (uint32_t)__builtin_amdgcn_readfirstlane((int)clear) : 0u);
       continue;
     }
     const int n_need = (int)__popcll(need);
diff --git a/raytracing_c_amd/csrc/rt_wavefront.hip b/raytracing_c_amd/csrc/rt_wavefront.hip
--- a/raytracing_c_amd/csrc/rt_wavefront.hip
+++ b/raytracing_c_amd/csrc/rt_wavefront.hip
@@ -149,7 +149,7 @@
         if (tile_open) {
           NewPath np = {0, 0, 0, 0};
           const bool got = regen_paths(T.phase, np, A->max_bounces > 0, U, tile_open, stopped, lane, tile_idx, n_chunks_tile, tile_x0, tile_y0,
-                                       shift, unit_paths, 0ull, no_time, w_paths);
+                                       shift, unit_paths, 0ull, no_time, w_paths, nullptr);
           if (got) {
             pix = np.pix;
             smp = np.sample;
diff --git a/raytracing_c_amd/ctypes_abi.py b/raytracing_c_amd/ctypes_abi.py
--- a/raytracing_c_amd/ctypes_abi.py
+++ b/raytracing_c_amd/ctypes_abi.py
@@ -242,7 +242,7 @@
     "rt_guided_variance_work_bytes", "rt_guided_denoise_variance", "rt_guided_denoise_variance_host", "rt_render_svgf",
     "rt_guided_upsample_work_bytes", "rt_guided_upsample", "rt_guided_upsample_host", "rt_render_upsampled",
     "rt_render_accumulate_chunks", "rt_adaptive_merge", "rt_resolve_adaptive", "rt_render_adaptive",
-    "rt_get_counters", "rt_get_skipped_root_visits", "rt_get_leafless_paths", "rt_get_triangleless_paths", "rt_get_fused_root_visits", "rt_get_shade_taps_form", "rt_materials_share_taps", "rt_last_kernel_ms", "rt_kernel_timing_reset", "rt_kernel_timing_mean_ms",
+    "rt_get_counters", "rt_get_skipped_root_visits", "rt_get_leafless_paths", "rt_get_triangleless_paths", "rt_get_clear_pair_paths", "rt_get_fused_root_visits", "rt_get_shade_taps_form", "rt_materials_share_taps", "rt_last_kernel_ms", "rt_kernel_timing_reset", "rt_kernel_timing_mean_ms",
 ]
 
 DIAG_ONLY_SYMBOLS = [
diff --git a/raytracing_c_amd/native.py b/raytracing_c_amd/native.py
--- a/raytracing_c_amd/native.py
+++ b/raytracing_c_amd/native.py
@@ -193,6 +193,8 @@
         d.rt_get_leafless_paths.argtypes = [P(C.c_uint64)]
     if hasattr(d, "rt_get_triangleless_paths"):
         d.rt_get_triangleless_paths.argtypes = [P(C.c_uint64)]
+    if hasattr(d, "rt_get_clear_pair_paths"):
+        d.rt_get_clear_pair_paths.argtypes = [P(C.c_uint64)]
     if hasattr(d, "rt_get_fused_root_visits"):
         d.rt_get_fused_root_visits.argtypes = [P(C.c_uint64)]
     if hasattr(d, "rt_get_shade_taps_form"):
diff --git a/raytracing_c_amd/tile_classes.py b/raytracing_c_amd/tile_classes.py
--- a/raytracing_c_amd/tile_classes.py
+++ b/raytracing_c_amd/tile_classes.py
@@ -9,10 +9,32 @@
     return min(n_nodes, max(room, 0))
 
 
+def _camera(cam_rows, width, height):
+    cam = np.asarray(cam_rows, F).reshape(-1, 4)[:3]
+    return cam, F(1.0) / F(width), F(1.0) / F(height), F(width) / F(height)
+
+
+def _planes(cam, focal_length, asp, ux0, ux1, uy0, uy1):
+    shape = np.broadcast(ux0, uy0).shape
+    c = np.zeros(shape + (4, 3), F)
+    for q in range(4):
+        cx = np.broadcast_to((ux1 if q in (1, 2) else ux0) * asp, shape)
+        cy = np.broadcast_to(-(uy1 if q >= 2 else uy0), shape)
+        cz = F(-focal_length)
+        for i in range(3):
+            c[..., q, i] = cam[i, 0] * cx + cam[i, 1] * cy + cam[i, 2] * cz
+    pn = np.zeros(shape + (4, 3), F)
+    for q in range(4):
+        n = np.cross(c[..., q, :], c[..., (q + 1) & 3, :]).astype(F)
+        flip = np.sum(n * c[..., (q + 2) & 3, :], axis=-1) > 0
+        n[flip] = -n[flip]
+        pn[..., q, :] = n
+    return pn
+
+
 def tile_pyramids(cam_rows, focal_length, width, height):
-    cam = np.asarray(cam_rows, F).reshape(-1, 4)[:3]
+    cam, inv_w, inv_h, asp = _camera(cam_rows, width, height)
     ty, tx = (height + 7) // 8, (width + 7) // 8
-    inv_w, inv_h, asp = F(1.0) / F(width), F(1.0) / F(height), F(width) / F(height)
     m = F(0.05)
     x0 = (np.arange(tx, dtype=F) * F(8))[None, :]
     y0 = (np.arange(ty, dtype=F) * F(8))[:, None]
@@ -20,20 +42,23 @@
     ux1 = (x0 + F(7.5) + m) * F(2.0) * inv_w - F(1.0)
     uy0 = (y0 - F(0.5) - m) * F(2.0) * inv_h - F(1.0)
     uy1 = (y0 + F(7.5) + m) * F(2.0) * inv_h - F(1.0)
-    c = np.zeros((ty, tx, 4, 3), F)
-    for q in range(4):
-        cx = np.broadcast_to((ux1 if q in (1, 2) else ux0) * asp, (ty, tx))
-        cy = np.broadcast_to(-(uy1 if q >= 2 else uy0), (ty, tx))
-        cz = F(-focal_length)
-        for i in range(3):
-            c[:, :, q, i] = cam[i, 0] * cx + cam[i, 1] * cy + cam[i, 2] * cz
-    pn = np.zeros((ty, tx, 4, 3), F)
-    for q in range(4):
-        n = np.cross(c[:, :, q], c[:, :, (q + 1) & 3]).astype(F)
-        flip = np.sum(n * c[:, :, (q + 2) & 3], axis=-1) > 0
-        n[flip] = -n[flip]
-        pn[:, :, q] = n
-    return pn, cam[:, 3].copy()
+    return _planes(cam, focal_length, asp, ux0, ux1, uy0, uy1), cam[:, 3].copy()
+
+
+def pair_pyramids(cam_rows, focal_length, width, height, rows=False):
+    cam, inv_w, inv_h, asp = _camera(cam_rows, width, height)
+    ty, tx = (height + 7) // 8, (width + 7) // 8
+    m = F(0.05)
+    p = np.arange(8 if rows else 32)
+    px = (np.zeros(8) if rows else 2 * (p & 3)).astype(F)[None, None, :]
+    py = (p if rows else p >> 2).astype(F)[None, None, :]
+    x = (np.arange(tx, dtype=F) * F(8))[None, :, None] + px
+    y = (np.arange(ty, dtype=F) * F(8))[:, None, None] + py
+    ux0 = (x - F(0.5) - m) * F(2.0) * inv_w - F(1.0)
+    ux1 = (x + F(7.5 if rows else 1.5) + m) * F(2.0) * inv_w - F(1.0)
+    uy0 = (y - F(0.5) - m) * F(2.0) * inv_h - F(1.0)
+    uy1 = (y + F(0.5) + m) * F(2.0) * inv_h - F(1.0)
+    return _planes(cam, focal_length, asp, ux0, ux1, uy0, uy1)
 
 
 def cull_masks(nodes, node_idx, pn, origin, margin=1e-3):
@@ -85,7 +110,8 @@
     return out
 
 
-def classify_tiles(nodes, depth, cam_rows, focal_length, width, height, margin=1e-3, give_up=64, tris=None, zero_culled=True):
+def classify_tiles(nodes, depth, cam_rows, focal_length, width, height, margin=1e-3, give_up=64, tris=None, zero_culled=True,
+                   pairs=None, pair_margin=None):
     nodes = np.asarray(nodes, F).reshape(-1, 6, 8)
     pn, origin = tile_pyramids(cam_rows, focal_length, width, height)
     ty, tx = pn.shape[:2]
@@ -99,6 +125,12 @@
     root_miss = np.zeros(n_tiles, bool)
     n_groups = np.zeros(n_tiles, np.int64)
     has_tri = np.zeros(n_tiles, bool)
+    ppn = blocked = None
+    if pairs:
+        ppn = pair_pyramids(cam_rows, focal_length, width, height, rows=pairs == "rows")
+        n_pairs = ppn.shape[2]
+        ppn = ppn.reshape(n_tiles, n_pairs, 4, 3)
+        blocked = np.zeros((n_tiles, n_pairs), bool)
     leaf0 = (8 ** max(depth, 0) - 1) // 7
     if leaf_level < 0 or len(nodes) == 0:
         reached_leaf[:] = True
@@ -121,10 +153,18 @@
                     pi, k = np.nonzero(surv)
                     np.add.at(n_groups, tile[pi], 1)
                     group = 8 * node[pi] + 1 + k - leaf0
-                    for a in range(0, len(pi), 1 << 15):
-                        b = slice(a, a + (1 << 15))
+                    step = 1 << (10 if pairs else 15)
+                    for a in range(0, len(pi), step):
+                        b = slice(a, a + step)
                         kept = ~cull_tris(tris, group[b], pn[tile[pi[b]]], origin, margin, zero_culled)
                         has_tri[tile[pi[b]][kept.any(axis=1)]] = True
+                        if pairs:
+                            r = np.nonzero(kept.any(axis=1))[0]
+                            t_r, g_r = tile[pi[b]][r], group[b][r]
+                            pc = cull_tris(tris, np.repeat(g_r, n_pairs), ppn[t_r].reshape(-1, 4, 3), origin,
+                                           margin if pair_margin is None else pair_margin, zero_culled)
+                            hit = (kept[r][:, None, :] & ~pc.reshape(len(r), n_pairs, 8)).any(axis=2)
+                            np.logical_or.at(blocked, t_r, hit)
                 break
             pi, k = np.nonzero(surv)
             tile, node = tile[pi], 8 * node[pi] + 1 + k
@@ -137,11 +177,36 @@
     if tris is not None:
         out.update(triangleless=((n_groups > 0) & ~has_tri).reshape(shape), n_groups=n_groups.reshape(shape),
                    n_entries=(n_listed - 1 + n_groups).reshape(shape))
+    if pairs:
+        out.update(clear=~blocked.reshape(shape + (-1,)))
     return out
 
 
-def classify_scene(hs, width, height, margin=1e-3, triangles=False, zero_culled=True):
+def clear_pair_masks(c, n_lds, cap=32, max_surv=4):
+    mixed = ~c["leafless"] & ~c["triangleless"] & (c["n_entries"] < cap) & (c["max_surv"] <= max_surv) & (c["max_node"] < n_lds)
+    return c["clear"] & mixed[..., None]
+
+
+def classify_scene(hs, width, height, margin=1e-3, triangles=False, zero_culled=True, pairs=None, pair_margin=None, give_up=64):
     cam = hs.scene.camera
     rows = [[cam.view_matrix.rows[i][j] for j in range(4)] for i in range(4)]
-    return classify_tiles(hs.nodes_array(), hs.depth, rows, cam.focal_length, width, height, margin,
-                          tris=hs.soa_array() if triangles else None, zero_culled=zero_culled)
+    return classify_tiles(hs.nodes_array(), hs.depth, rows, cam.focal_length, width, height, margin, give_up,
+                          tris=hs.soa_array() if triangles or pairs else None, zero_culled=zero_culled, pairs=pairs, pair_margin=pair_margin)
+
+
+def unit_decode(u, n_sb, clear=0):
+    clear &= 0xFFFFFFFF
+    if clear == 0:
+        grp, pair = u >> 2, u & 3
+        row, sb = divmod(grp, n_sb)
+        return 4 * row + pair, sb, False
+    n_clear = bin(clear).count("1") * n_sb
+    is_clear = u < n_clear
+    v, m = (u, clear) if is_clear else (u - n_clear, ~clear & 0xFFFFFFFF)
+    j, sb = divmod(v, n_sb)
+    p = [b for b in range(32) if (m >> b) & 1][j]
+    return p, sb, is_clear
+
+
+def pair_mask_words(clear):
+    return (np.asarray(clear, np.uint64) << np.arange(32, dtype=np.uint64)).sum(axis=-1).astype(np.uint32)
```

After: 24480 Mray/s. No clear change (-0.0%).
